# TravisWheelerLab/AvxWindowFmIndex

Hardware: AMD Instinct MI355X
Metric: Mkmers/sec located, GRCh38 nucleotide index (higher is better)
Workload: dtype u64

## Files before the change

### avxwindowfmindex_amd/_lib.py

```python
import ctypes as C
import os
import subprocess

_HERE = os.path.dirname(os.path.abspath(__file__))
LIB_PATH = os.environ.get("AWFM_LIB_PATH") or os.path.join(_HERE, "libawfmindex_amd.so")
_LIB = None

AwFmAlphabetAmino, AwFmAlphabetDna, AwFmAlphabetRna = 1, 2, 3
AwFmSuccess, AwFmFileReadOkay, AwFmFileWriteOkay = 1, 2, 3
AwFmGeneralFailure = -1
AwFmIllegalPositionError = -6
AwFmUnsupportedVersionError = -2
AwFmFileReadFail = -11

API_SYMBOLS = [
    "awFmCreateIndex", "awFmCreateIndexFromFasta", "awFmDeallocIndex", "awFmWriteIndexToFile",
    "awFmReadIndexFromFile", "awFmCreateKmerSearchList", "awFmDeallocKmerSearchList", "awFmParallelSearchLocate",
    "awFmParallelSearchCount", "awFmFindSearchRangeForString", "awFmReadSequenceFromFile",
    "awFmCreateInitialQueryRange", "awFmCreateInitialQueryRangeFromChar",
    "awFmNucleotideIterativeStepBackwardSearch", "awFmAminoIterativeStepBackwardSearch",
    "awFmFindDatabaseHitPositions", "awFmFindDatabaseHitPositionSingle",
    "awFmGetLocalSequencePositionFromIndexPosition", "awFmNucleotideBacktraceReturnPreviousLetterIndex",
    "awFmAminoBacktraceReturnPreviousLetterIndex", "awFmGetHeaderStringFromSequenceNumber", "awFmSearchRangeLength",
    "awFmReturnCodeIsFailure", "awFmReturnCodeIsSuccess", "awFmGetNumSequences",
]
GPU_SYMBOLS = [
    "awfmGpuDeviceCount", "awfmGpuLastError", "awfmGpuIndexCreate", "awfmGpuIndexDestroy", "awfmGpuIndexAcquire", "awfmGpuIndexAcquireAll",
    "awfmGpuIndexRelease", "awfmGpuIndexDeviceBytes", "awfmGpuIndexDevice", "awfmGpuIndexSetKernel", "awfmGpuIndexSetWide", "awfmGpuIndexIsWide", "awfmGpuLastBatchStatus", "awfmGpuIndexSetDeepSeed", "awfmGpuIndexSetDenseSa", "awfmGpuPinnedBuffer", "awfmGpuLocateHostWindows", "awfmGpuLocateWindow", "awfmGpuAosLock",
    "awfmGpuAosUnlock", "awfmGpuSearch", "awfmGpuSearchHits", "awfmGpuSearchHitsSparse", "awfmGpuIndexSetOrdered", "awfmGpuSearchHitsIsOrdered", "awfmGpuLastOrderedKernelMs", "awfmGpuLastOrderedKernelIsLookup", "awfmGpuLastOrderedKept", "awfmGpuLastSecondWindow",
    "awfmGpuScanScratchBytes", "awfmGpuHitOffsets", "awfmGpuHitOffsetsFromCounts", "awfmGpuLocate", "awfmGpuCountHost", "awfmGpuLocateHost",
    "awfmGpuCreateIndex", "awfmGpuSearchTally", "awfmGpuSynthText", "awfmGpuSynthRandomQueries", "awfmGpuSynthPlantedQueries",
    "awfmGpuSynthMixedLengths", "awfmGpuSynthMixedQueries", "awfmGpuSynthGenomeText", "awfmGpuSynthPlantedQueriesClean",
    "awfmPackKmers", "awfmGpuPackKmers", "awfmGpuUnpackKmers", "awfmGpuHostAlloc", "awfmGpuHostFree", "awfmGpuStreamPacked",
    "awfmGpuStreamChars", "awfmGpuCountPackedHost", "awfmGpuLocatePackedHost", "awfmGpuIndexSetPairImage", "awfmGpuIndexHasPairImage",
    "awfmGpuSearchHitsPacked", "awfmGpuLocateTo", "awfmGpuSearchHitsLineTally", "awfmGpuIndexDeepSeedK", "awfmGpuSearchHitsCompact", "awfmGpuCompactHits", "awfmGpuSortHits",
    "awfmGpuStreamPackedSparse", "awfmGpuStreamCharsSparse", "awfmGpuSearchHitsInOrder", "awfmGpuSearchHitsInOrderCounts",
    "awfmGpuSortHitsOnDevice", "awfmGpuHitOffsetsOnDevice", "awfmGpuLocateOnDevice", "awfmGpuLastOrderedSearchKernelMs", "awfmGpuOrderedKernelLog", "awfmGpuIndexDeepSeedBuildSeconds", "awfmGpuIndexDeepSeedTransientBytes", "awfmGpuIndexHasDenseSa", "awfmGpuIndexDenseSaBuildSeconds", "awfmGpuIndexLengthTableBytes", "awfmGpuIndexLengthTableBuildSeconds", "awfmGpuMixedLookupLineTally",
    "awfmGpuListLocateOnDevice", "awfmGpuLastLookupFront", "awfmGpuLastSearchWasExactLookup", "awfmGpuSynthPlantedQueriesUnique", "awfmGpuStreamRetire", "awfmGpuIndexDescribe", "awfmGpuIndexDeepSeedAllocSeconds", "awfmGpuAosLastStages", "awfmHostCopyGBs",
    "awfmLocalPositions", "awfmGpuIndexSetRecordTable", "awfmGpuIndexNumRecords", "awfmGpuLocalPositions", "awfmGpuLocateHostLocal",
    "awfmLongestSuffixMatches", "awfmGpuLongestSuffixMatches", "awfmOneSubstitutionSearch", "awfmGpuOneSubstitutionSearch",
    "awfmReadCandidates", "awfmGpuReadCandidates", "awfmGpuReadCandidatesScratchBytes",
    "awfmReadChains", "awfmGpuReadChains", "awfmGpuReadChainsScratchBytes",
    "awfmGpuIndexSetText", "awfmGpuIndexTextLength", "awfmTextWindows", "awfmGpuTextWindows", "awfmVerifyChains", "awfmGpuVerifyChains",
    "awfmAlignChains", "awfmGpuAlignChainsScratchBytes", "awfmGpuAlignChains",
    "awfmAlignChainsAffine", "awfmGpuAlignChainsAffineScratchBytes", "awfmGpuAlignChainsAffine",
    "awfmScoreChainsAffine", "awfmGpuScoreChainsAffine",
    "awfmScoreWindowsAffine", "awfmGpuScoreWindowsAffineScratchBytes", "awfmGpuScoreWindowsAffine",
    "awfmGpuOrderBuckets", "awfmGpuOrderKmers", "awfmGpuSearchOrderedRecords", "awfmGpuSearchOrderedRecordsCounts", "awfmGpuSearchGeneralRecords", "awfmGpuMergeBucketRuns",
]
CHUNK_SINK = C.CFUNCTYPE(C.c_int, C.c_void_p, C.c_uint64, C.c_uint64, C.POINTER(C.c_uint32), C.POINTER(C.c_uint64), C.c_uint64)


SPARSE_CHUNK_SINK = C.CFUNCTYPE(C.c_int, C.c_void_p, C.c_uint64, C.c_uint64, C.c_uint64, C.POINTER(C.c_uint32), C.POINTER(C.c_uint64),
                                C.POINTER(C.c_uint64), C.c_uint64)
HIT_WINDOW_SINK = C.CFUNCTYPE(C.c_int, C.c_void_p, C.c_uint64, C.c_uint64, C.c_uint64, C.c_uint64, C.POINTER(C.c_uint64))


class AwFmIndexConfiguration(C.Structure):
    _fields_ = [("suffixArrayCompressionRatio", C.c_uint8), ("kmerLengthInSeedTable", C.c_uint8),
                ("alphabetType", C.c_int), ("keepSuffixArrayInMemory", C.c_bool), ("storeOriginalSequence", C.c_bool)]


class AwFmCompressedSuffixArray(C.Structure):
    _fields_ = [("valueBitWidth", C.c_uint8), ("values", C.POINTER(C.c_uint8)), ("compressedByteLength", C.c_uint64)]


class AwFmSearchRange(C.Structure):
    _fields_ = [("startPtr", C.c_uint64), ("endPtr", C.c_uint64)]


class AwFmCandidateInputs(C.Structure):
    _fields_ = [("readSeedOffsets", C.c_void_p), ("numSeeds", C.c_uint64), ("seedEnds", C.c_void_p), ("seedLengths", C.c_void_p),
                ("fixedLength", C.c_uint32), ("hitOffsets", C.c_void_p), ("numHits", C.c_uint64), ("positions", C.c_void_p),
                ("sequenceNumbers", C.c_void_p)]


class AwFmCandidateOutputs(C.Structure):
    _fields_ = [("sequences", C.c_void_p), ("diagonals", C.c_void_p), ("votes", C.c_void_p), ("diagonalSpans", C.c_void_p),
                ("readBegins", C.c_void_p), ("readEnds", C.c_void_p), ("numCandidates", C.c_void_p), ("keptHits", C.c_void_p),
                ("numOverflowed", C.c_void_p)]


# ... 84 lines not shown
        import torch
    except Exception:
        pass
    L = C.CDLL(LIB_PATH, mode=C.RTLD_GLOBAL)
    IP, LP = C.POINTER(AwFmIndex), C.POINTER(AwFmKmerSearchList)
    RP = C.POINTER(AwFmSearchRange)
    vp, u64 = C.c_void_p, C.c_uint64
    sig = {
        "awFmCreateIndex": (C.c_int, [C.POINTER(IP), C.POINTER(AwFmIndexConfiguration), vp, C.c_size_t, C.c_char_p]),
        "awFmCreateIndexFromFasta": (C.c_int, [C.POINTER(IP), C.POINTER(AwFmIndexConfiguration), C.c_char_p, C.c_char_p]),
        "awFmDeallocIndex": (None, [IP]),
        "awFmWriteIndexToFile": (C.c_int, [IP, vp, u64, C.c_char_p]),
        "awFmReadIndexFromFile": (C.c_int, [C.POINTER(IP), C.c_char_p, C.c_bool]),
        "awFmCreateKmerSearchList": (LP, [C.c_size_t]),
        "awFmDeallocKmerSearchList": (None, [LP]),
        "awFmParallelSearchLocate": (C.c_int, [IP, LP, C.c_uint32]),
        "awFmParallelSearchCount": (None, [IP, LP, C.c_uint32]),
        "awFmFindSearchRangeForString": (AwFmSearchRange, [IP, C.c_char_p, C.c_size_t]),
        "awFmReadSequenceFromFile": (C.c_int, [IP, C.c_size_t, C.c_size_t, C.c_char_p]),
        "awFmCreateInitialQueryRange": (AwFmSearchRange, [IP, C.c_char_p, u64]),
        "awFmCreateInitialQueryRangeFromChar": (AwFmSearchRange, [IP, C.c_char]),
        "awFmNucleotideIterativeStepBackwardSearch": (None, [IP, RP, C.c_uint8]),
        "awFmAminoIterativeStepBackwardSearch": (None, [IP, RP, C.c_uint8]),
        "awFmFindDatabaseHitPositions": (C.POINTER(u64), [IP, RP, C.POINTER(C.c_int)]),
        "awFmFindDatabaseHitPositionSingle": (u64, [IP, u64, C.POINTER(C.c_int)]),
        "awFmNucleotideBacktraceReturnPreviousLetterIndex": (C.c_uint8, [IP, C.POINTER(u64)]),
        "awFmAminoBacktraceReturnPreviousLetterIndex": (C.c_uint8, [IP, C.POINTER(u64)]),
        "awFmGetLocalSequencePositionFromIndexPosition": (C.c_int, [IP, C.c_size_t, C.POINTER(C.c_size_t),
                                                                   C.POINTER(C.c_size_t)]),
        "awFmGetHeaderStringFromSequenceNumber": (C.c_int, [IP, C.c_size_t, C.POINTER(C.c_char_p), C.POINTER(C.c_size_t)]),
        "awFmSearchRangeLength": (C.c_size_t, [RP]),
        "awFmReturnCodeIsFailure": (C.c_bool, [C.c_int]),
        "awFmReturnCodeIsSuccess": (C.c_bool, [C.c_int]),
        "awFmGetNumSequences": (C.c_uint32, [IP]),
        "awfmGpuDeviceCount": (C.c_int, []),
        "awfmGpuLastError": (C.c_char_p, []),
        "awfmGpuIndexCreate": (C.c_int, [IP, C.c_int, C.POINTER(vp)]),
        "awfmGpuIndexDestroy": (None, [vp]),
        "awfmGpuIndexAcquire": (vp, [IP]),
        "awfmGpuIndexAcquireAll": (C.c_int, [IP, C.POINTER(vp), C.c_int]),
        "awfmGpuIndexRelease": (None, [IP]),
        "awfmGpuIndexDeviceBytes": (u64, [vp]),
        "awfmGpuIndexDevice": (C.c_int, [vp]),
        "awfmGpuIndexSetKernel": (None, [vp, C.c_int]),
        "awfmGpuIndexSetWide": (None, [vp, C.c_int]),
        "awfmGpuIndexIsWide": (C.c_int, [vp]),
        "awfmGpuLastBatchStatus": (C.c_int, []),
        "awfmGpuIndexSetOrdered": (None, [vp, C.c_int]),
        "awfmGpuSearchHitsIsOrdered": (C.c_int, [vp, C.c_int, C.c_uint32, u64]),
        "awfmGpuLastOrderedKernelMs": (C.c_double, [vp]),
        "awfmGpuLastOrderedKernelIsLookup": (C.c_int, [vp]),
        "awfmGpuLastOrderedKept": (C.c_uint64, [vp]),
        "awfmGpuLastSecondWindow": (None, [vp, C.POINTER(C.c_uint64 * 2)]),
        "awfmGpuIndexSetDeepSeed": (C.c_int, [vp, C.c_uint]),
        "awfmGpuIndexSetDenseSa": (C.c_int, [vp, C.c_int]),
        "awfmGpuIndexSetPairImage": (C.c_int, [vp, C.c_int]),
        "awfmGpuIndexHasPairImage": (C.c_int, [vp]),
        "awfmGpuIndexDeepSeedK": (C.c_uint, [vp]),
        "awfmGpuIndexDeepSeedBuildSeconds": (C.c_double, [vp]),
        "awfmGpuIndexDeepSeedTransientBytes": (u64, [vp]),
        "awfmGpuIndexHasDenseSa": (C.c_int, [vp]),
        "awfmGpuIndexDenseSaBuildSeconds": (C.c_double, [vp]),
        "awfmGpuIndexLengthTableBytes": (u64, [vp]),
        "awfmGpuIndexLengthTableBuildSeconds": (C.c_double, [vp]),
        "awfmGpuMixedLookupLineTally": (C.c_int, [vp, vp, vp, u64, C.POINTER(u64 * 8)]),
        "awfmGpuSearch": (C.c_int, [vp, vp, vp, C.c_uint32, u64, vp, vp, vp]),
        "awfmGpuSearchHits": (C.c_int, [vp, vp, vp, C.c_uint32, u64, vp, vp, vp]),
        "awfmGpuSearchHitsSparse": (C.c_int, [vp, vp, vp, C.c_uint32, u64, vp, vp, vp]),
        "awfmGpuSearchHitsCompact": (C.c_int, [vp, vp, vp, C.c_uint32, u64, C.c_int, vp, vp, C.c_uint32, vp, vp]),
        "awfmGpuCompactHits": (C.c_int, [vp, vp, vp, u64, vp, vp, vp, vp, C.c_uint32, vp, vp]),
        "awfmGpuSearchHitsInOrder": (C.c_int, [vp, vp, vp, C.c_uint32, u64, C.c_int, vp, vp, vp]),
        "awfmGpuSearchHitsInOrderCounts": (C.c_int, [vp, vp, vp, C.c_uint32, u64, C.c_int, vp, vp, vp, vp]),
        "awfmGpuOrderBuckets": (C.c_uint32, [vp, C.c_uint32, u64]),
        "awfmGpuOrderKmers": (C.c_int, [vp, vp, C.c_uint32, u64, u64, u64, vp, vp, vp]),
        "awfmGpuSearchOrderedRecords": (C.c_int, [vp, vp, vp, C.c_uint32, C.c_uint32, C.c_uint32, u64, vp, vp, vp]),
        "awfmGpuSearchOrderedRecordsCounts": (C.c_int, [vp, vp, vp, C.c_uint32, C.c_uint32, C.c_uint32, u64, vp, vp, vp, vp]),
        "awfmGpuMergeBucketRuns": (C.c_int, [vp, vp, vp, vp, C.c_uint32, C.c_uint32, C.c_uint32, C.c_uint32, vp, vp, vp]),
        "awfmGpuSearchGeneralRecords": (C.c_int, [vp, vp, C.c_uint32, u64, u64, u64, vp, vp, vp, vp, vp]),
        "awfmGpuSortHits": (C.c_int, [vp, vp, vp, C.c_uint32, vp]),
        "awfmGpuSortHitsOnDevice": (C.c_int, [vp, vp, vp, C.c_uint32, vp, u64, vp]),
        "awfmGpuListLocateOnDevice": (C.c_int, [vp, vp, vp, C.c_uint32, vp, u64, vp, vp, vp, u64, vp, vp]),
        "awfmGpuLastLookupFront": (C.c_int, [vp]),
        "awfmGpuLastSearchWasExactLookup": (C.c_int, [vp]),
        "awfmGpuStreamRetire": (None, [vp, vp]),
        "awfmGpuIndexDescribe": (C.c_int, [vp, C.c_char_p, C.c_int]),
        "awfmGpuIndexDeepSeedAllocSeconds": (C.c_double, [vp]),
        "awfmGpuAosLastStages": (None, [C.POINTER(C.c_double * 10)]),
        "awfmHostCopyGBs": (C.c_double, [C.c_uint32, u64]),
        "awfmGpuHitOffsetsOnDevice": (C.c_int, [vp, vp, vp, u64, vp, vp, vp]),
        "awfmGpuLocateOnDevice": (C.c_int, [vp, vp, vp, u64, u64, vp, vp]),
        "awfmGpuLastOrderedSearchKernelMs": (C.c_double, [vp]),
        "awfmGpuOrderedKernelLog": (C.c_int, [vp, C.POINTER(C.c_double), C.POINTER(C.c_double), C.c_int]),
        "awfmGpuScanScratchBytes": (u64, [u64]),
        "awfmGpuHitOffsets": (C.c_int, [vp, vp, u64, vp, vp, C.POINTER(u64), vp]),
        "awfmGpuHitOffsetsFromCounts": (C.c_int, [vp, vp, u64, vp, vp, C.POINTER(u64), vp]),
        "awfmGpuLocate": (C.c_int, [vp, vp, vp, u64, u64, vp, vp]),
        "awfmGpuLocateTo": (C.c_int, [vp, vp, vp, u64, u64, vp, vp, vp]),
        "awfmGpuLocateWindow": (C.c_int, [vp, vp, vp, u64, u64, u64, u64, vp, vp, vp]),
        "awfmGpuLocateHostWindows": (C.c_int, [vp, vp, vp, C.c_uint32, u64, vp, vp, HIT_WINDOW_SINK, vp]),
        "awfmGpuCountHost": (C.c_int, [vp, vp, vp, C.c_uint32, u64, vp, vp]),
        "awfmGpuLocateHost": (C.c_int, [vp, vp, vp, C.c_uint32, u64, vp, vp, C.POINTER(C.POINTER(u64))]),
        "awfmLocalPositions": (C.c_int, [IP, vp, u64, vp, vp, C.POINTER(u64), C.c_uint]),
        "awfmLongestSuffixMatches": (C.c_int, [IP, vp, vp, vp, C.c_uint32, u64, C.c_uint32, vp, vp, vp, C.c_uint]),
        "awfmGpuLongestSuffixMatches": (C.c_int, [vp, vp, vp, vp, C.c_uint32, u64, C.c_uint32, vp, vp, vp, vp]),
        "awfmOneSubstitutionSearch": (C.c_int, [IP, vp, vp, C.c_uint32, u64, C.c_int, vp, vp, vp, u64, vp, vp, vp, C.c_uint]),
        "awfmGpuOneSubstitutionSearch": (C.c_int, [vp, vp, vp, C.c_uint32, u64, C.c_int, vp, vp, vp, u64, vp, vp, vp, vp]),
# ... 77 lines not shown
```

### avxwindowfmindex_amd/api.py

```python
import ctypes as C
import os

import numpy as np

from . import _lib
from ._lib import (AwFmAlphabetAmino, AwFmAlphabetDna, AwFmAlphabetRna, AwFmFileReadOkay, AwFmFileWriteOkay,
                   AwFmIllegalPositionError, AwFmSuccess, AwFmUnsupportedVersionError)

ILLEGAL_SEQUENCE = 0xFFFFFFFF


class AwFmError(RuntimeError):
    def __init__(self, what, rc):
        msg = _lib.lib().awfmGpuLastError().decode(errors="replace")
        super().__init__(f"{what} failed with AwFmReturnCode {rc}" + (f": {msg}" if msg else ""))
        self.rc = rc


def _check(what, rc, ok=(AwFmSuccess, AwFmFileReadOkay, AwFmFileWriteOkay)):
    if rc not in ok:
        raise AwFmError(what, rc)
    return rc


# ... 745 lines not shown
            _check("awfmGpuIndexCreate", L.awfmGpuIndexCreate(index.ptr, device, C.byref(h)))
            self.handle = h
        self.index = index

    @classmethod
    def acquire_all(cls, index, max_handles=8):
        L = _lib.lib()
        if L.awfmGpuDeviceCount() <= 0:
            raise RuntimeError("no HIP device: the search path is GPU only (no CPU fallback)")
        handles = (C.c_void_p * max_handles)()
        n = L.awfmGpuIndexAcquireAll(index.ptr, handles, max_handles)
        out = []
        for h in handles[:n]:
            g = cls.__new__(cls)
            g.owned, g.handle, g.index = False, C.c_void_p(h), index
            out.append(g)
        return out

    @property
    def device_bytes(self):
        return int(_lib.lib().awfmGpuIndexDeviceBytes(self.handle))

    def set_deep_seed(self, deep_k):
        _check("awfmGpuIndexSetDeepSeed", _lib.lib().awfmGpuIndexSetDeepSeed(self.handle, deep_k))

    @property
    def deep_seed_k(self):
        return int(_lib.lib().awfmGpuIndexDeepSeedK(self.handle))

    @property
    def deep_seed_build(self):
        L = _lib.lib()
        return float(L.awfmGpuIndexDeepSeedBuildSeconds(self.handle)), int(L.awfmGpuIndexDeepSeedTransientBytes(self.handle))

    @property
    def deep_seed_alloc_s(self):
        return float(_lib.lib().awfmGpuIndexDeepSeedAllocSeconds(self.handle))

    def set_dense_sa(self, enable=True):
        _check("awfmGpuIndexSetDenseSa", _lib.lib().awfmGpuIndexSetDenseSa(self.handle, int(bool(enable))))

    @property
    def has_dense_sa(self):
        return bool(_lib.lib().awfmGpuIndexHasDenseSa(self.handle))

    @property
    def dense_sa_build_s(self):
        return float(_lib.lib().awfmGpuIndexDenseSaBuildSeconds(self.handle))

    @property
    def length_tables(self):
        return (int(_lib.lib().awfmGpuIndexLengthTableBytes(self.handle)), float(_lib.lib().awfmGpuIndexLengthTableBuildSeconds(self.handle)))

    def mixed_lookup_line_tally(self, d_chars, d_offsets, n):
        out = (C.c_uint64 * 8)()
        _check("awfmGpuMixedLookupLineTally", _lib.lib().awfmGpuMixedLookupLineTally(self.handle, d_chars, d_offsets, n, C.byref(out)))
        keys = ("length_table_lines", "deep_table_lines", "pair_level_lines", "nuc_level_lines", "kmers_alive_after_the_table",
                "kmers_with_hits", "general_kmers", "block_reads_executed")
        return {k: int(v) for k, v in zip(keys, out)}

    def set_pair_image(self, enable=True):
        _check("awfmGpuIndexSetPairImage", _lib.lib().awfmGpuIndexSetPairImage(self.handle, int(bool(enable))))

    @property
    def has_pair_image(self):
        return bool(_lib.lib().awfmGpuIndexHasPairImage(self.handle))

    def set_kernel(self, kernel):
        _lib.lib().awfmGpuIndexSetKernel(self.handle, kernel)

    def set_wide(self, wide=True):
        _lib.lib().awfmGpuIndexSetWide(self.handle, int(bool(wide)))

    @property
    def is_wide(self):
        return bool(_lib.lib().awfmGpuIndexIsWide(self.handle))

    def set_record_table(self, ends):
        ends = np.ascontiguousarray(ends, dtype=np.uint64)
        _check("awfmGpuIndexSetRecordTable", _lib.lib().awfmGpuIndexSetRecordTable(self.handle, ends.ctypes.data if ends.size else None,
                                                                                   ends.size))

    @property
    def num_records(self):
        return int(_lib.lib().awfmGpuIndexNumRecords(self.handle))

    def local_positions(self, d_positions, capacity, d_seq, d_local, d_num_positions=0, d_num_illegal=0, stream=0):
        _check("awfmGpuLocalPositions", _lib.lib().awfmGpuLocalPositions(self.handle, d_positions or None, capacity, d_num_positions or None,
                                                                         d_seq or None, d_local or None, d_num_illegal or None, stream or None))

    def read_candidates(self, inputs, num_reads, outputs, d_scratch, max_hits_per_seed=0, band=0, min_votes=1, max_candidates=4, stream=0):
        _check("awfmGpuReadCandidates", _lib.lib().awfmGpuReadCandidates(
            self.handle, C.byref(inputs), num_reads, max_hits_per_seed, band, min_votes, max_candidates, C.byref(outputs),
            d_scratch or None, stream or None))

    def read_chains(self, inputs, num_reads, d_sequences, d_diagonals, d_spans, outputs, d_scratch, max_hits_per_seed=0, band=0,
                    max_candidates=4, lookback=CHAINS_MAX_LOOKBACK, gap_penalty=0, stream=0):
        _check("awfmGpuReadChains", _lib.lib().awfmGpuReadChains(
            self.handle, C.byref(inputs), num_reads, max_hits_per_seed, band, max_candidates, d_sequences or None, d_diagonals or None,
            d_spans or None, lookback, gap_penalty, C.byref(outputs), d_scratch or None, stream or None))

    def set_text(self, text):
        if text is None:
            t = np.zeros(0, np.uint8)
        else:
            t = np.frombuffer(text, np.uint8) if isinstance(text, (bytes, bytearray)) else np.ascontiguousarray(text, dtype=np.uint8)
# ... 268 lines not shown

    def describe(self):
        import ctypes as C
        buf = C.create_string_buffer(2048)
        _lib.lib().awfmGpuIndexDescribe(self.handle, buf, 2048)
        return buf.value.decode()

    def stream_retire(self, stream):
        _lib.lib().awfmGpuStreamRetire(self.handle, stream or None)

    def last_lookup_front(self):
        return int(_lib.lib().awfmGpuLastLookupFront(self.handle))

    def last_search_was_exact_lookup(self):
        return bool(_lib.lib().awfmGpuLastSearchWasExactLookup(self.handle))

    def list_locate_on_device(self, d_hit_kmers, d_hit_ranges, capacity, d_num_hits, n, d_sorted_kmers, d_sorted_ranges, d_hit_offsets,
                              capacity_hits, d_positions, stream=0):
        _check("awfmGpuListLocateOnDevice", _lib.lib().awfmGpuListLocateOnDevice(
            self.handle, d_hit_kmers, d_hit_ranges, capacity, d_num_hits, n, d_sorted_kmers, d_sorted_ranges, d_hit_offsets,
            capacity_hits, d_positions or None, stream or None))

    def hit_offsets_on_device(self, d_counts, d_ranges, n, d_hit_offsets, d_scratch, stream=0):
        _check("awfmGpuHitOffsetsOnDevice", _lib.lib().awfmGpuHitOffsetsOnDevice(self.handle, d_counts or None, d_ranges or None, n,
                                                                                 d_hit_offsets, d_scratch, stream or None))

    def locate_on_device(self, d_ranges, d_hit_offsets, n, capacity_hits, d_positions, stream=0):
        _check("awfmGpuLocateOnDevice", _lib.lib().awfmGpuLocateOnDevice(self.handle, d_ranges, d_hit_offsets, n, capacity_hits,
                                                                         d_positions, stream or None))

    def ordered_kernel_log(self, max_entries=1024):
        front = (C.c_double * max_entries)()
        kern = (C.c_double * max_entries)()
        n = _lib.lib().awfmGpuOrderedKernelLog(self.handle, front, kern, max_entries)
        return [(front[i], kern[i]) for i in range(n)]

    def last_ordered_search_kernel_ms(self):
        return float(_lib.lib().awfmGpuLastOrderedSearchKernelMs(self.handle))

    def search_hits_is_ordered(self, has_offsets, fixed_length, n):
        return bool(_lib.lib().awfmGpuSearchHitsIsOrdered(self.handle, int(bool(has_offsets)), fixed_length, n))

    def last_ordered_kernel_ms(self):
        return float(_lib.lib().awfmGpuLastOrderedKernelMs(self.handle))

    def last_ordered_kept(self):
        return int(_lib.lib().awfmGpuLastOrderedKept(self.handle))

    def last_second_window(self):
        out = (C.c_uint64 * 2)()
        _lib.lib().awfmGpuLastSecondWindow(self.handle, C.byref(out))
        return int(out[0]), int(out[1])

    def last_ordered_kernel_is_lookup(self):
        return bool(_lib.lib().awfmGpuLastOrderedKernelIsLookup(self.handle))

    def set_ordered(self, mode):
        _lib.lib().awfmGpuIndexSetOrdered(self.handle, mode)

    def search_tally(self, d_chars, d_offsets, fixed_length, n):
        out = (C.c_uint64 * 4)()
        _check("awfmGpuSearchTally", _lib.lib().awfmGpuSearchTally(self.handle, d_chars, d_offsets or None, fixed_length,
                                                                   n, C.byref(out)))
        return {"seeded": int(out[0]), "steps": int(out[1]), "blocks": int(out[2]), "chars": int(out[3])}

    def search_hits_line_tally(self, d_chars, d_offsets, fixed_length, n):
        out = (C.c_uint64 * 8)()
        _check("awfmGpuSearchHitsLineTally", _lib.lib().awfmGpuSearchHitsLineTally(self.handle, d_chars, d_offsets or None,
                                                                                   fixed_length, n, C.byref(out)))
        keys = ("seed_table_lines", "deep_table_lines", "pair_level_lines", "nuc_level_lines", "ordered_kmers",
                "record_bytes_per_kmer", "kmers_with_hits", "general_kmers")
        return {k: int(v) for k, v in zip(keys, out)}

    def hit_offsets(self, d_ranges, n, d_hit_offsets, d_scratch, stream=0):
        total = C.c_uint64(0)
        _check("awfmGpuHitOffsets", _lib.lib().awfmGpuHitOffsets(self.handle, d_ranges, n, d_hit_offsets, d_scratch,
                                                                 C.byref(total), stream or None))
        return int(total.value)

    def hit_offsets_from_counts(self, d_counts, n, d_hit_offsets, d_scratch, stream=0):
        total = C.c_uint64(0)
        _check("awfmGpuHitOffsetsFromCounts", _lib.lib().awfmGpuHitOffsetsFromCounts(
            self.handle, d_counts, n, d_hit_offsets, d_scratch, C.byref(total), stream or None))
        return int(total.value)

    def locate(self, d_ranges, d_hit_offsets, n, total_hits, d_positions, stream=0):
        _check("awfmGpuLocate", _lib.lib().awfmGpuLocate(self.handle, d_ranges, d_hit_offsets, n, total_hits,
                                                         d_positions, stream or None))

    def locate_window(self, d_ranges, d_hit_offsets, query_begin, query_end, hit_begin, hit_end, d_positions, stream=0):
        _check("awfmGpuLocateWindow", _lib.lib().awfmGpuLocateWindow(self.handle, d_ranges, d_hit_offsets, query_begin, query_end,
                                                                     hit_begin, hit_end, d_positions, d_positions, stream or None))

    @staticmethod
    def scan_scratch_bytes(n):
        return int(_lib.lib().awfmGpuScanScratchBytes(n))

    def destroy(self):
        if self.handle:
            if self.owned:
                _lib.lib().awfmGpuIndexDestroy(self.handle)
            self.handle = None

    def __del__(self):
        try:
            self.destroy()
# ... 3 lines not shown
```

### avxwindowfmindex_amd/csrc/awfm_device.h

```cpp
#ifndef AWFM_DEVICE_H
#define AWFM_DEVICE_H

#include <hip/hip_runtime.h>

#include <atomic>
#include <cstdlib>
#include <cstring>
#include <mutex>
#include <shared_mutex>
#include <thread>
#include <vector>
#include <string>

#include "awfm_internal.h"

void awfmGpuSetError(const char *what);
void awfmGpuSetHipError(const char *what, hipError_t e);

namespace {

inline void setError(const char *what, hipError_t e) { awfmGpuSetHipError(what, e); }
inline void setError(const char *what) { awfmGpuSetError(what); }

#define AWFM_HIP_TRY(call, failRc)                      \
// ... 699 lines not shown
      if (half) {
        const unsigned pm = kAminoTables.planeMask[letter];
        for (unsigned j = 0; j < 4; j++) {
          Piece lo, hi;
          lo.x = planeWord(0, j);
          lo.y = planeWord(1, j);
          lo.z = planeWord(2, j);
          lo.w = planeWord(3, j);
          hi.x = planeWord(4, j);
          hi.y = hi.z = hi.w = 0;
          count += __popc(aminoOccSlice(lo, hi, pm & 0xFFu, pm >> 8));
        }
      }
      count -= super[(blk >> (kAminoSuperShift - kBlockShift)) * kAminoSuperStride + letter];
    }
    c16[s] = (unsigned)count & 0xFFFFu;
  }
  out[(blk * kSlices + k) * 2ull] = make_uint4(b[0], b[1], b[2], b[3]);
  out[(blk * kSlices + k) * 2ull + 1ull] = make_uint4(b[4], c16[0] | (c16[1] << 16), c16[2] | (c16[3] << 16), c16[4] | (c16[5] << 16));
  unsigned sentinelBits = ~(b[0] | b[1] | b[2] | b[3] | b[4]);
  while (sentinelBits) {
    const unsigned bit = (unsigned)(__ffs((int)sentinelBits) - 1);
    sentinelBits &= sentinelBits - 1u;
    const unsigned long long pos = (blk << kBlockShift) + k * 32u + bit;
    if (pos < bwtLength) *sentinelPos = pos;
  }
}

}

struct AwFmGpuIndex;

struct AwFmGpuImage {
  DevIndex dev{};
  void *dBlocks = nullptr;
  void *dSuper = nullptr;
  void *dSeed = nullptr;
  void *dSa = nullptr;
  void *dPrefix = nullptr;
  void *dDeepSeed = nullptr;
  uint64_t deepSeedBytes = 0;
  double deepSeedBuildSeconds = 0.0;
  double deepSeedAllocSeconds = 0.0;
  uint64_t deepSeedTransientBytes = 0;
  void *dDeepBig = nullptr;
  std::mutex lengthMutex;
  void *dLengthTable = nullptr;
  unsigned lengthDepths = 0;
  bool lengthTried = false;
  unsigned lengthRetryIn = 0;
  void *dLengthBig = nullptr;
  uint64_t lengthTableBytes = 0;
  double lengthTableBuildSeconds = 0.0;
  void *dDenseSa = nullptr;
  bool denseWide = false;
  uint64_t denseSaBytes = 0;
  double denseSaBuildSeconds = 0.0;
  void *dPairBlocks = nullptr, *dPairSuper = nullptr, *dPairSuper32 = nullptr, *dPairC = nullptr;
  uint64_t pairBytes = 0;
  std::string accelNotes;
  uint64_t deviceBytes = 0;
  uint64_t numBlocks = 0;
  std::mutex joinMutex;
  std::thread accelThread;
  std::atomic<int> accelState{0};
  struct PendingAccel {
    void *deepTable = nullptr, *deepBig = nullptr;
    uint64_t deepBytes = 0, deepBigBytes = 0, deepTransient = 0;
    unsigned deepK = 0, deepFormat = 0, deepNext = 0, numDeepBig = 0;
    double deepSeconds = 0.0, deepAllocSeconds = 0.0;
    void *dense = nullptr;
    bool denseWide = false;
    uint64_t denseBytes = 0;
    double denseSeconds = 0.0;
    std::string notes;
  } pendingAccel;
  std::mutex streamMutex;
  struct AwFmGpuStreamState *streamState = nullptr;
  std::mutex handlesMutex;
  std::vector<AwFmGpuIndex *> handles;
  std::shared_mutex recordMutex;
  DevRecords records{};
  void *dRecords = nullptr;
  uint64_t recordBytes = 0;
  bool recordsInLds = false;
  unsigned recordLdsBytes = 0;
  unsigned recordGrid = 0;
  void *dText = nullptr;
  uint64_t textLength = 0;
  uint64_t textBytes = 0;
};

struct AwFmGpuIndex {
  AwFmGpuImage *image = nullptr;
  int lane = 0;
  int device = 0;
  bool amino = false;
  int numCUs = 256;
  AwFmGpuKernel kernel = AWFM_GPU_KERNEL_AUTO;
  bool forceWide = false;
  std::mutex workMutex;
  void *dWork = nullptr;
  size_t workBytes = 0;
  void *dHits = nullptr;
  size_t hitsBytes = 0;
  mutable uint64_t hitBudgetAuto = 0;
  void *dSparse = nullptr;
  size_t sparseBytes = 0;
  hipEvent_t windowEvent[2] = {nullptr, nullptr};
  int orderMode = -1;
  std::mutex orderMutex;
  struct StreamGate {
    hipEvent_t done = nullptr;
    bool recorded = false;
    bool pending = false;
    hipStream_t lastStream = nullptr;
    std::thread::id lastThread;
  };
  struct OrderSlot {
    void *mem = nullptr;
    size_t bytes = 0;
    StreamGate gate;
    unsigned long long lastUse = 0;
    int prepParity = -1;
  };
  static constexpr int kOrderSlots = 2;
  OrderSlot orderSlot[kOrderSlots];
  unsigned long long orderUses = 0;
  int orderCur = 0;
  int orderPrevParity = -1;
  void *dOrder = nullptr;
  size_t orderBytes = 0;
  hipEvent_t orderDoneEvent = nullptr;
  bool orderDoneArmed = false;
  StreamGate sparseGate;
  hipEvent_t orderTiming[4] = {nullptr, nullptr, nullptr, nullptr};
  bool orderTimedFront = false, orderTimedKernel = false;
  struct OrderLogEntry {
    hipEvent_t ev[4] = {nullptr, nullptr, nullptr, nullptr};
    bool front = false, kernel = false;
  };
  static constexpr unsigned kOrderLogMax = 1024;
  std::vector<OrderLogEntry> orderLog;
  unsigned long long orderLogCount = 0;
  int orderLookup = 0;
  const unsigned *orderSampleAt = nullptr;
  unsigned orderSamples = 0;
  bool orderLookupFused = false;
  const unsigned *orderFusedKeptAt = nullptr;
  const unsigned *orderKeptAt = nullptr;
  struct LookupPredict {
    unsigned long long *verdictHost = nullptr;
    unsigned searches = 0;
    int lastFront = -1;
    unsigned lastJudged = 0;
    unsigned holdoff = 0;
    unsigned holdoffNext = 8;
    unsigned agreed = 0;
  } predict;
  int lastSearchExact = 0;
  std::mutex aosMutex;
  void *pinned[4] = {nullptr, nullptr, nullptr, nullptr};
  size_t pinnedBytes[4] = {0, 0, 0, 0};
};

inline const char *awfmGpuDiag(const char *key) {
  const char *env = awfmKnob(AWFM_KNOB_DIAG);
  if (!env) return nullptr;
  static thread_local char value[32];
  const size_t keyLen = strlen(key);
  for (const char *at = env; *at;) {
    const char *end = strchr(at, ',');
    const size_t len = end ? (size_t)(end - at) : strlen(at);
    if (len > keyLen && !strncmp(at, key, keyLen) && at[keyLen] == '=') {
      const size_t n = len - keyLen - 1 < sizeof(value) - 1 ? len - keyLen - 1 : sizeof(value) - 1;
      memcpy(value, at + keyLen + 1, n);
      value[n] = 0;
      return value;
    }
    at += len + (end ? 1 : 0);
  }
  return nullptr;
}

inline uint64_t awfmDeviceBlocks(uint64_t bwtLength) { return 2 * awfmNumBlocks(bwtLength); }
inline uint64_t awfmDeviceBlockBytes(bool amino) { return amino ? 128 : 64; }
inline unsigned awfmSuperShift(bool amino, uint64_t bwtLength) {
  if (amino) return kAminoSuperShift;
  if (const char *env = awfmGpuDiag("nuc_super_shift")) {
    if (!strcmp(env, "auto")) {
      unsigned shift = 13;
      while (((bwtLength - 1) >> shift) + 1 > 48) shift++;
      return shift < kNucSuperShift ? shift : kNucSuperShift;
    }
    const int v = atoi(env);
    if (v >= 13 && v < (int)kNucSuperShift) return (unsigned)v;
  }
  return kNucSuperShift;
}
inline uint64_t awfmNumSuper(uint64_t bwtLength, bool amino, unsigned superShift) {
  (void)amino;
  return ((bwtLength - 1) >> superShift) + 1;
}
// ... 125 lines not shown
```

### avxwindowfmindex_amd/csrc/awfm_gpu_image.hip

```cpp
#include <hip/hip_runtime.h>
#include <cstdio>
#include <cstdlib>
#include <cstring>
#include <mutex>
#include <string>
#include <system_error>
#include <vector>

#include "awfm_device.h"
#include "awfm_search_kernel.h"
#include "awfm_locate_kernel.h"

thread_local hipStream_t awfmGpuSetupStream = nullptr;
static thread_local std::string tlsError;
void awfmGpuSetError(const char *what) { tlsError = what; }
void awfmGpuSetHipError(const char *what, hipError_t e) { tlsError = std::string(what) + ": " + hipGetErrorString(e); }


namespace {

std::mutex tableMutex;
struct ImageEntry {
  const AwFmIndex *index;
  AwFmGpuIndex *handle;
// ... 335 lines not shown
    if (!take(h->aosMutex) || !take(h->workMutex) || !take(h->orderMutex)) return;
  held = true;
}
AwFmGpuExclusive::~AwFmGpuExclusive() {
  while (!locked.empty()) {
    locked.back()->unlock();
    locked.pop_back();
  }
}

void awfmGpuAdoptAccelerators(AwFmGpuImage *image, bool wait) {
  if (image->accelState.load() == 0) return;
  if (wait) joinBuilder(image);
  else if (image->accelState.load() != 2) return;
  AwFmGpuExclusive section(image, wait);
  if (!section.held || image->accelState.load() != 2) return;
  joinBuilder(image);
  AwFmGpuImage::PendingAccel &from = image->pendingAccel;
  if (from.deepTable) installDeepSeed(image, &from);
  if (from.dense) {
    image->dDenseSa = from.dense;
    image->denseWide = from.denseWide;
    image->denseSaBytes = from.denseBytes;
    image->denseSaBuildSeconds = from.denseSeconds;
    from.dense = nullptr;
  }
  image->accelNotes += from.notes;
  from.notes.clear();
  image->accelState.store(0);
}
extern "C" {

void awfmGpuIndexDestroy(AwFmGpuIndex *g) {
  if (!g) return;
  AwFmGpuImage *image = g->image;
  if (g->lane) {
    std::lock_guard<std::mutex> lock(image->handlesMutex);
    for (size_t i = 0; i < image->handles.size(); i++)
      if (image->handles[i] == g) {
        image->handles.erase(image->handles.begin() + (long)i);
        break;
      }
  } else {
    joinBuilder(image);
  }
  {
    DeviceGuard guard(g->device);
    if (!g->lane) {
      if (image->pendingAccel.deepTable) (void)hipFree(image->pendingAccel.deepTable);
      if (image->pendingAccel.deepBig) (void)hipFree(image->pendingAccel.deepBig);
      if (image->pendingAccel.dense) (void)hipFree(image->pendingAccel.dense);
      awfmGpuStreamStateFree(image);
      void *owned[] = {image->dBlocks, image->dSuper, image->dSeed, image->dSa, image->dPrefix, image->dDeepSeed, image->dDeepBig,
                       image->dDenseSa, image->dLengthTable, image->dLengthBig, image->dPairBlocks, image->dPairSuper,
                       image->dPairSuper32, image->dPairC, image->dRecords, image->dText};
      for (void *p : owned)
        if (p) (void)hipFree(p);
    }
    if (g->dWork) (void)hipFree(g->dWork);
    if (g->dHits) (void)hipFree(g->dHits);
    for (auto &slot : g->orderSlot) {
      if (slot.mem) (void)hipFree(slot.mem);
      if (slot.gate.done) (void)hipEventDestroy(slot.gate.done);
    }
    if (g->dSparse) (void)hipFree(g->dSparse);
    if (g->sparseGate.done) (void)hipEventDestroy(g->sparseGate.done);
    for (auto &entry : g->orderLog)
      for (int i = 0; i < 4; i++)
        if (entry.ev[i]) (void)hipEventDestroy(entry.ev[i]);
    for (int i = 0; i < 2; i++)
      if (g->windowEvent[i]) (void)hipEventDestroy(g->windowEvent[i]);
    for (int i = 0; i < 4; i++)
      if (g->pinned[i]) (void)hipHostFree(g->pinned[i]);
    if (g->predict.verdictHost) (void)hipHostFree(g->predict.verdictHost);
  }
  if (!g->lane) delete image;
  delete g;
}

static int aosDevices(int *devs, int maxOut) {
  int n = 0;
  const char *env = awfmKnob(AWFM_KNOB_DEVICES);
  if (env && !strcmp(env, "all")) {
    const int count = awfmGpuDeviceCount();
    for (int d = 0; d < count && n < maxOut; d++) devs[n++] = d;
  } else if (env && *env) {
    for (const char *c = env; *c && n < maxOut;) {
      devs[n++] = atoi(c);
      while (*c && *c != ',') c++;
      if (*c == ',') c++;
    }
  }
  if (n == 0) {
    devs[n++] = -1;
    for (int lane = 1; lane < 3 && n < maxOut; lane++) devs[n++] = -1;
  }
  return n;
}

static AwFmGpuIndex *addLane(AwFmGpuIndex *primary) {
  AwFmGpuIndex *g = new AwFmGpuIndex();
  g->image = primary->image;
  g->device = primary->device;
  g->amino = primary->amino;
  g->numCUs = primary->numCUs;
  g->kernel = primary->kernel;
  g->forceWide = primary->forceWide;
// ... 38 lines not shown
  return n;
}

AwFmGpuIndex *awfmGpuIndexAcquire(const struct AwFmIndex *index) {
  AwFmGpuIndex *g = nullptr;
  if (awfmGpuIndexAcquireAll(index, &g, 1) != 1) return nullptr;
  awfmGpuAdoptAccelerators(g->image, true);
  return g;
}

void awfmGpuIndexRelease(const struct AwFmIndex *index) {
  std::vector<AwFmGpuIndex *> doomed;
  {
    std::lock_guard<std::mutex> lock(tableMutex);
    for (size_t i = 0; i < imageTable.size();) {
      if (imageTable[i].index == index) {
        doomed.push_back(imageTable[i].handle);
        imageTable.erase(imageTable.begin() + (long)i);
      } else {
        i++;
      }
    }
  }
  for (AwFmGpuIndex *g : doomed)
    if (g->lane) awfmGpuIndexDestroy(g);
  for (AwFmGpuIndex *g : doomed)
    if (!g->lane) awfmGpuIndexDestroy(g);
}

void *awfmGpuPinnedBuffer(AwFmGpuIndex *g, int slot, uint64_t bytes) {
  if (!g || slot < 0 || slot > 3) return nullptr;
  if (bytes <= g->pinnedBytes[slot]) return g->pinned[slot];
  DeviceGuard guard(g->device);
  if (g->pinned[slot]) (void)hipHostFree(g->pinned[slot]);
  g->pinned[slot] = nullptr;
  g->pinnedBytes[slot] = 0;
  const size_t want = bytes + bytes / 4 + 4096;
  if (hipHostMalloc(&g->pinned[slot], want, hipHostMallocDefault) != hipSuccess) {
    setError("awfmGpuPinnedBuffer: hipHostMalloc failed");
    g->pinned[slot] = nullptr;
    return nullptr;
  }
  g->pinnedBytes[slot] = want;
  return g->pinned[slot];
}
void awfmGpuAosLock(AwFmGpuIndex *g) {
  if (g) g->aosMutex.lock();
}
void awfmGpuAosUnlock(AwFmGpuIndex *g) {
  if (g) g->aosMutex.unlock();
}

static uint64_t imageBytes(const AwFmGpuImage *image) {
  return image->deviceBytes + image->deepSeedBytes + image->denseSaBytes + image->pairBytes + image->lengthTableBytes + image->recordBytes + image->textBytes;
}
uint64_t awfmGpuIndexDeviceBytes(const AwFmGpuIndex *g) { return g && !g->lane ? imageBytes(g->image) : 0; }

static enum AwFmReturnCode applyDeepSeed(AwFmGpuIndex *g, unsigned deepK);

enum AwFmReturnCode awfmGpuIndexSetDeepSeed(AwFmGpuIndex *g, unsigned deepK) {
  if (!g) {
    setError("awfmGpuIndexSetDeepSeed: null image");
    return AwFmNullPtrError;
  }
  if (g->lane) {
    setError("awfmGpuIndexSetDeepSeed: set it on the primary image, not on a lane");
    return AwFmIllegalPositionError;
  }
  awfmGpuAdoptAccelerators(g->image, true);
  DeviceGuard guard(g->device);
  AwFmGpuExclusive section(g->image);
  return applyDeepSeed(g, deepK);
}

static enum AwFmReturnCode buildDeepSeed(AwFmGpuIndex *g, unsigned deepK, AwFmGpuImage::PendingAccel *to) {
  void *table = nullptr, *big = nullptr;
  uint64_t bytes = 0, peak = 0;
  unsigned format = 0, numBig = 0;
  struct timespec t0, t1;
  clock_gettime(CLOCK_MONOTONIC, &t0);
  if (!awfmGpuBuildDeepSeedTable(g, deepK, &table, &bytes, &peak, &to->deepAllocSeconds, &format, &big)) return AwFmGeneralFailure;
  const int next = awfmGpuDeepSeedAddNext(g, table, deepK, format, &big, &numBig);
  (void)awfmGpuSetupSync();
  clock_gettime(CLOCK_MONOTONIC, &t1);
  if (next < 0) {
    (void)hipFree(table);
    if (big) (void)hipFree(big);
    return AwFmGeneralFailure;
  }
  to->deepTable = table;
  to->deepBig = big;
  to->deepBytes = bytes;
  to->deepBigBytes = !big ? 0u
                     : format == 2u ? ((g->image->dev.bwtLength >> (g->amino ? kAminoWideBigShift : kDeepWideBigShift)) + 2u) * 8u
                                    : ((g->image->dev.bwtLength >> (g->amino ? kAminoDeepBigShift : kDeepBigShift)) + 5u) * 4u;
  to->deepTransient = peak > bytes ? peak - bytes : 0;
  to->deepK = deepK;
  to->deepFormat = format;
  to->deepNext = next > 0 ? 1u : 0u;
  to->numDeepBig = numBig;
  to->deepSeconds = (double)(t1.tv_sec - t0.tv_sec) + 1e-9 * (double)(t1.tv_nsec - t0.tv_nsec);
  if (awfmKnob(AWFM_KNOB_VERBOSE))
    fprintf(stderr, "[awfm deeper table] depth %u, entry format %u: %.2f GB in %.2f s; next-step bits %s; %u entries with long ranges\n", deepK, format,
            (double)bytes * 1e-9, to->deepSeconds, next > 0 ? "yes" : "no", numBig);
  return AwFmSuccess;
}
static void installDeepSeed(AwFmGpuImage *image, AwFmGpuImage::PendingAccel *from) {
  image->dDeepSeed = from->deepTable;
  image->dDeepBig = from->deepBig;
  image->deepSeedBytes = from->deepBytes + from->deepBigBytes;
  image->deepSeedBuildSeconds = from->deepSeconds;
  image->deepSeedAllocSeconds = from->deepAllocSeconds;
  image->deepSeedTransientBytes = from->deepTransient;
  image->dev.deepSeed = (const ulonglong2 *)from->deepTable;
  image->dev.deepNarrow = from->deepFormat;
  image->dev.deepNext = from->deepNext;
  image->dev.numDeepBig = from->numDeepBig;
  image->dev.deepBigBySp = (const unsigned *)from->deepBig;
  image->dev.deepK = from->deepTable ? from->deepK : 0u;
  from->deepTable = from->deepBig = nullptr;
}

static enum AwFmReturnCode applyDeepSeed(AwFmGpuIndex *g, unsigned deepK) {
  AwFmGpuImage *image = g->image;
  (void)hipDeviceSynchronize();
  if (image->dDeepSeed) (void)hipFree(image->dDeepSeed);
  if (image->dDeepBig) (void)hipFree(image->dDeepBig);
  {
    std::lock_guard<std::mutex> lock(image->lengthMutex);
    if (image->dLengthTable) (void)hipFree(image->dLengthTable);
    if (image->dLengthBig) (void)hipFree(image->dLengthBig);
    image->dLengthTable = nullptr;
    image->dLengthBig = nullptr;
    image->lengthDepths = 0;
    image->lengthTableBytes = 0;
    image->lengthTried = false;
  }
  AwFmGpuImage::PendingAccel built;
  enum AwFmReturnCode rc = AwFmSuccess;
  if (deepK != 0) {
    image->dev.deepSeed = nullptr;
    image->dev.deepK = 0;
    rc = buildDeepSeed(g, deepK, &built);
  }
  installDeepSeed(image, &built);
  return rc;
}

static unsigned chooseDeepSeedK(const AwFmGpuIndex *g, std::string &notes);
static enum AwFmReturnCode applyDeepSeedFromEnv(AwFmGpuIndex *g) {
  const unsigned deepK = chooseDeepSeedK(g, g->image->accelNotes);
  if (deepK == 0) return AwFmSuccess;
  DeviceGuard guard(g->device);
  return applyDeepSeed(g, deepK);
}
static unsigned chooseDeepSeedK(const AwFmGpuIndex *g, std::string &notes) {
  int deepK = 0;
  if (const char *env = awfmKnob(g->amino ? AWFM_KNOB_AMINO_DEEP_SEED_K : AWFM_KNOB_DEEP_SEED_K)) {
    deepK = atoi(env);
  } else if (g->amino) {
// ... 39 lines not shown
    (void)awfmGpuApplyPairImage(g, false);
    g->image->accelNotes += "pair image: not built (no device memory for 1 byte per position); ";
  }
  return rc;
}

enum AwFmReturnCode awfmGpuIndexSetPairImage(AwFmGpuIndex *g, int enable) {
  if (!g) {
    setError("awfmGpuIndexSetPairImage: null image");
    return AwFmNullPtrError;
  }
  if (g->lane) {
    setError("awfmGpuIndexSetPairImage: set it on the primary image, not on a lane");
    return AwFmIllegalPositionError;
  }
  awfmGpuAdoptAccelerators(g->image, true);
  DeviceGuard guard(g->device);
  AwFmGpuExclusive section(g->image);
  const enum AwFmReturnCode rc = awfmGpuApplyPairImage(g, enable != 0);
  if (rc != AwFmSuccess) (void)awfmGpuApplyPairImage(g, false);
  return rc;
}
int awfmGpuIndexHasPairImage(const AwFmGpuIndex *g) { return g && g->image->dev.pairBlocks ? 1 : 0; }
unsigned awfmGpuIndexDeepSeedK(const AwFmGpuIndex *g) { return g ? g->image->dev.deepK : 0u; }
double awfmGpuIndexDeepSeedAllocSeconds(const AwFmGpuIndex *g) { return g ? g->image->deepSeedAllocSeconds : 0.0; }
double awfmGpuIndexDeepSeedBuildSeconds(const AwFmGpuIndex *g) { return g ? g->image->deepSeedBuildSeconds : 0.0; }
uint64_t awfmGpuIndexDeepSeedTransientBytes(const AwFmGpuIndex *g) { return g ? g->image->deepSeedTransientBytes : 0; }

int awfmGpuIndexDevice(const AwFmGpuIndex *g) { return g ? g->device : -1; }
void awfmGpuIndexSetKernel(AwFmGpuIndex *g, enum AwFmGpuKernel kernel) {
  if (g) g->kernel = kernel;
}
int awfmGpuIndexIsWide(const AwFmGpuIndex *g) { return g && !awfmImageNarrow(g) ? 1 : 0; }
void awfmGpuIndexSetWide(AwFmGpuIndex *g, int wide) {
  if (!g) return;
  if (g->lane) {
    g->forceWide = wide != 0;
    return;
  }
  std::lock_guard<std::mutex> lock(g->image->handlesMutex);
  for (AwFmGpuIndex *h : g->image->handles) h->forceWide = wide != 0;
}


int awfmGpuIndexDescribe(const AwFmGpuIndex *g, char *out, int outBytes) {
  if (!g || !out || outBytes <= 0) return 0;
  const AwFmGpuImage *image = g->image;
  std::string text = std::string(g->amino ? "amino" : "nucleotide") + " image of " + std::to_string(image->dev.bwtLength) + " positions, " +
                     std::to_string(imageBytes(image)) + " bytes on device " + std::to_string(g->device) + ": ";
  if (!g->amino) text += image->dev.pairBlocks ? "pair image yes; " : "pair image no; ";
  text += image->dev.deepK ? "deeper table depth " + std::to_string(image->dev.deepK) + (image->dev.deepNext ? " with next-step bits; " : "; ") : "deeper table no; ";
  text += image->dDenseSa ? "full suffix array yes; " : "full suffix array no; ";
  if (!g->amino) text += image->dLengthTable ? "tables per k-mer length 1.." + std::to_string(image->lengthDepths) + "; " : "tables per k-mer length not built (the first large mixed-length batch builds them); ";
  text += awfmGpuDescribeRecordTable(image);
  text += awfmGpuDescribeText(image);
  if (!image->accelNotes.empty()) text += "notes: " + image->accelNotes;
  while (!text.empty() && (text.back() == ' ' || text.back() == ';')) text.pop_back();
  const int n = (int)text.size() < outBytes - 1 ? (int)text.size() : outBytes - 1;
  memcpy(out, text.data(), (size_t)n);
  out[n] = 0;
  return (int)text.size();
}
uint64_t awfmGpuIndexLengthTableBytes(const AwFmGpuIndex *g) { return g ? g->image->lengthTableBytes : 0; }
double awfmGpuIndexLengthTableBuildSeconds(const AwFmGpuIndex *g) { return g ? g->image->lengthTableBuildSeconds : 0.0; }

}
```

### avxwindowfmindex_amd/csrc/awfm_gpu_ordered.hip

```cpp
#include <cstring>
#include <cstdio>
#include <cstdlib>
#include <cstddef>

#include <hip/hip_runtime.h>
#include <hip/hip_ext.h>
#include <rocprim/rocprim.hpp>

#include "awfm_ordered_kernel.h"
#include "awfm_amino_lookup_kernel.h"
#include "awfm_count_order_kernel.h"

namespace {

inline size_t alignUp256(size_t v) { return (v + 255) / 256 * 256; }

__global__ void __launch_bounds__(256) fillSparseKernel(unsigned *__restrict__ kmers, ulonglong2 *__restrict__ ranges, unsigned cap,
                                                        unsigned *__restrict__ count) {
  const unsigned i = blockIdx.x * 256u + threadIdx.x;
  if (i < cap) {
    kmers[i] = 0xFFFFFFFFu;
    ranges[i] = make_ulonglong2(1ull, 0ull);
  }
  if (i == 0) *count = 0u;
}
inline hipError_t fillSparseList(const SparseOut *sparse, hipStream_t s) {
  if (!sparse || !sparse->count) return hipSuccess;
  hipLaunchKernelGGL(fillSparseKernel, dim3((sparse->cap + 255u) / 256u), dim3(256), 0, s, sparse->kmers, sparse->ranges, sparse->cap, sparse->count);
  return hipGetLastError();
}
constexpr size_t kOrderCounterBytes = 131072;
static_assert(256 + 8 * kTicketGroups * 8 * 256 <= kOrderCounterBytes, "ticket counters");

template <class Kernel>
unsigned residentGrid(const AwFmGpuIndex *g, Kernel kernel, size_t dynamicLds = 0, int threads = kThreads) {
  int perCU = 0;
  if (hipOccupancyMaxActiveBlocksPerMultiprocessor(&perCU, kernel, threads, dynamicLds) != hipSuccess || perCU < 1) perCU = 4;
  if (perCU > 8) perCU = 8;
  return (unsigned)g->numCUs * (unsigned)perCU;
}

inline bool pairSteps(const AwFmGpuIndex *g) { return g->image->dev.pairBlocks != nullptr; }

template <bool NARROW, bool VARLEN, bool PAIR = false, bool TOUCH = false, bool BUCKET = false, bool LIST = false>
enum AwFmReturnCode launchOrderedKernel(AwFmGpuIndex *g, hipStream_t s, uint32_t len, unsigned depth, const ulonglong2 *table,
                                        unsigned long long nq, const void *recs, const unsigned *generalCount, ulonglong2 *rng,
                                        uint32_t *dCounts, const OrderTouch *touch = nullptr, const unsigned *bucketStart = nullptr,
                                        const BucketFormat bucketFmt = BucketFormat(), const SparseOut *sparse = nullptr,
                                        const unsigned *skipSampleAlive = nullptr, unsigned skipSamples = 0u) {
  constexpr int G = 4;
  const bool superInLds = PAIR && NARROW && awfmPairSuperInLds(g);
  const size_t lds = superInLds ? (size_t)g->image->dev.numPairSuper * 64u : 0u;
  DevIndex dev = g->image->dev;
  dev.pairSuperInLds = superInLds ? 1u : 0u;
  constexpr int threads = orderedThreads(PAIR);
  unsigned grid = residentGrid(g, orderedSearchKernel<G, NARROW, VARLEN, PAIR, TOUCH, BUCKET, LIST>, lds, threads);
  const unsigned long long blocks = (nq + threads / G - 1) / (threads / G);
  if (blocks < grid) grid = (unsigned)blocks;
  if (grid >= 8u) grid &= ~7u;
  const bool timed = g->orderTiming[2] != nullptr;
  OrderSkip<VARLEN> skip;
  if constexpr (VARLEN) {
    skip.sampleAlive = skipSampleAlive;
    skip.samples = skipSamples;
  }
  AWFM_LAUNCH_WITH_EVENTS((orderedSearchKernel<G, NARROW, VARLEN, PAIR, TOUCH, BUCKET, LIST>), dim3(grid ? grid : 1u), dim3(threads), (unsigned)lds, s,
                        timed ? g->orderTiming[2] : nullptr, timed ? g->orderTiming[3] : nullptr, dev, recs, nq, generalCount, len, depth, table,
                        rng, dCounts, (unsigned *)generalCount + 64, touch ? *touch : OrderTouch(), bucketStart, bucketFmt,
                        sparse ? *sparse : SparseOut(),
                        BUCKET ? 2u : 1u, skip);
  AWFM_HIP_TRY(hipGetLastError(), AwFmGeneralFailure);
  g->orderTimedKernel = timed;
  if (timed) g->orderLog[(g->orderLogCount - 1u) % AwFmGpuIndex::kOrderLogMax].kernel = true;
  return AwFmSuccess;
}

template <bool NARROW, bool CSR>
enum AwFmReturnCode launchLeftover(AwFmGpuIndex *g, hipStream_t s, const uint8_t *dChars, const unsigned long long *off, uint32_t len,
                                   unsigned long long nq, ulonglong2 *rng, uint32_t *dCounts, const void *recs, unsigned recordBytes,
                                   unsigned indexAt, const unsigned *leftCount, const SparseOut *sparse, bool last = true) {
  const unsigned grid = residentGrid(g, searchKernel<false, 4, CSR, false, NARROW, true>);
  AWFM_LAUNCH_WITH_EVENTS((searchKernel<false, 4, CSR, false, NARROW, true>), dim3(grid), dim3(kThreads), 0u, s, nullptr, last ? g->orderDoneEvent : nullptr,
                          g->image->dev, dChars, off, len, nq, rng, dCounts, (unsigned long long *)nullptr, (const unsigned char *)recs, recordBytes,
                          indexAt, nq, leftCount, sparse ? *sparse : SparseOut(), (const unsigned *)nullptr, 0u);
  AWFM_HIP_TRY(hipGetLastError(), AwFmGeneralFailure);
  if (last) g->orderDoneArmed = g->orderDoneEvent != nullptr;
  return AwFmSuccess;
}

template <bool NARROW, bool VARLEN>
enum AwFmReturnCode launchOrdered(AwFmGpuIndex *g, hipStream_t s, const uint8_t *dChars, const unsigned long long *off,
                                  uint32_t len, unsigned depth, const ulonglong2 *table, unsigned long long nq,
                                  const void *recs, const unsigned *generalCount, ulonglong2 *rng, uint32_t *dCounts,
                                  const OrderTouch *touch = nullptr, const SparseOut *sparse = nullptr,
                                  const unsigned *skipSampleAlive = nullptr, unsigned skipSamples = 0u) {
  enum AwFmReturnCode rc;
  const BucketFormat none = BucketFormat();
  if (touch)
    rc = pairSteps(g) ? launchOrderedKernel<NARROW, VARLEN, true, true>(g, s, len, depth, table, nq, recs, generalCount, rng, dCounts, touch)
                      : launchOrderedKernel<NARROW, VARLEN, false, true>(g, s, len, depth, table, nq, recs, generalCount, rng, dCounts, touch);
  else
    rc = pairSteps(g) ? launchOrderedKernel<NARROW, VARLEN, true>(g, s, len, depth, table, nq, recs, generalCount, rng, dCounts, nullptr, nullptr, none, sparse, skipSampleAlive, skipSamples)
                      : launchOrderedKernel<NARROW, VARLEN, false>(g, s, len, depth, table, nq, recs, generalCount, rng, dCounts, nullptr, nullptr, none, sparse, skipSampleAlive, skipSamples);
  if (rc != AwFmSuccess) return rc;
  return launchLeftover<NARROW, VARLEN>(g, s, dChars, off, len, nq, rng, dCounts, recs, (unsigned)sizeof(QueryRec), (unsigned)offsetof(QueryRec, index),
                                        generalCount, sparse);
}

template <bool NARROW>
enum AwFmReturnCode launchBucketed(AwFmGpuIndex *g, hipStream_t s, const uint8_t *dChars, uint32_t len, unsigned depth,
                                   const ulonglong2 *table, unsigned long long nq, const void *recs, const unsigned *bucketStart,
                                   const BucketFormat &fmt, const unsigned *generalCount, ulonglong2 *rng, uint32_t *dCounts,
                                   bool packed, const OrderTouch *touch, const SparseOut *sparse, bool countRecords = false) {
  const bool pair = pairSteps(g);
  enum AwFmReturnCode rc;
  if (touch)
    rc = pair ? launchOrderedKernel<NARROW, false, true, true, true>(g, s, len, depth, table, nq, recs, generalCount, rng, dCounts, touch, bucketStart, fmt)
              : launchOrderedKernel<NARROW, false, false, true, true>(g, s, len, depth, table, nq, recs, generalCount, rng, dCounts, touch, bucketStart, fmt);
  else if (sparse && sparse->count)
    rc = pair ? launchOrderedKernel<NARROW, false, true, false, true, true>(g, s, len, depth, table, nq, recs, generalCount, rng, dCounts, nullptr, bucketStart, fmt, sparse)
              : launchOrderedKernel<NARROW, false, false, false, true, true>(g, s, len, depth, table, nq, recs, generalCount, rng, dCounts, nullptr, bucketStart, fmt, sparse);
  else
    rc = pair ? launchOrderedKernel<NARROW, false, true, false, true>(g, s, len, depth, table, nq, recs, generalCount, rng, dCounts, nullptr, bucketStart, fmt, sparse)
              : launchOrderedKernel<NARROW, false, false, false, true>(g, s, len, depth, table, nq, recs, generalCount, rng, dCounts, nullptr, bucketStart, fmt, sparse);
  if (rc != AwFmSuccess || packed || countRecords) return rc;
  return launchLeftover<NARROW, false>(g, s, dChars, nullptr, len, nq, rng, dCounts, recs, 8u, 0u, generalCount, sparse);
}

}

static bool orderedApplies(const AwFmGpuIndex *g, bool hasOffsets, uint32_t fixedLength, unsigned long long nq,
                           unsigned *depthOut, const ulonglong2 **tableOut) {
  if (g->amino || nq >= 0xFFFFFFFFull || g->image->dev.seedK == 0 || g->image->dev.seedK >= 32 || g->image->dev.deepK >= 32) return false;
  if (!hasOffsets) {
    if (fixedLength == 0 || fixedLength > 32) return false;
    const bool deep = g->image->dev.deepK != 0 && fixedLength >= g->image->dev.deepK;
    const unsigned depth = deep ? g->image->dev.deepK : g->image->dev.seedK;
    if (fixedLength < depth) return false;
    if (depthOut) *depthOut = depth;
    if (tableOut) *tableOut = deep ? g->image->dev.deepSeed : g->image->dev.seed;
  }
  int mode = g->orderMode;
  if (mode < 0) {
    if (const char *env = awfmKnob(AWFM_KNOB_ORDERED)) mode = atoi(env) != 0;
  }
  if (mode < 0) {
    mode = nq >= (1ull << 23) && g->image->dev.bwtLength >= (1ull << 28);
  }
  return mode != 0;
}

int awfmGpuDeepSeedAddNext(AwFmGpuIndex *g, void *table, unsigned deepK, unsigned format, void **bigOut, unsigned *numBigOut) {
  *numBigOut = 0;
  if (!g || !table || format == 0u || deepK == 0) return 0;
  if (g->amino ? deepK > 7u : (!g->image->dev.pairBlocks || deepK > 16u)) return 0;
  if (awfmKnob(AWFM_KNOB_DEEP_NEXT) && atoi(awfmKnob(AWFM_KNOB_DEEP_NEXT)) == 0) return 0;
  DeviceGuard guard(g->device);
  if (format == 2u) {
    unsigned *dCount = nullptr;
    if (hipMalloc((void **)&dCount, 16) != hipSuccess) {
      (void)hipGetLastError();
      return 0;
    }
    unsigned numBig = 0;
    bool ok = awfmGpuSetupMemset(dCount, 0, 16) == hipSuccess;
    if (ok) {
      DevIndex dev = g->image->dev;
      dev.deepNarrow = 2u;
      dev.deepBigBySp = (const unsigned *)*bigOut;
      dev.pairSuperInLds = 0u;
      if (g->amino) {
        unsigned long long numEntries = 1;
        for (unsigned k = 0; k < deepK; k++) numEntries *= 20ull;
        const unsigned grid = residentGrid(g, aminoDeepNextKernel<false>, 0, kThreads);
        hipLaunchKernelGGL(aminoDeepNextKernel<false>, dim3(grid ? grid : 1u), dim3(kThreads), 0, awfmGpuSetupStream, dev, (uint2 *)table, numEntries, (unsigned *)nullptr, dCount);
      } else {
// ... 344 lines not shown
                          const unsigned *sampleAlive = nullptr, unsigned samples = 0u) {
  launchEncode4At<32u>(len, grid, lds, s, dChars, fmt, nq, codes, hist, binsPad, sampleAlive, samples);
}

template <unsigned K, bool NARROW>
static void launchLookupSearchAt(unsigned len, unsigned grid, size_t lds, hipStream_t s, const DevIndex &dev, const uint8_t *dChars,
                                 const BucketFormat &fmt, unsigned useNext, unsigned long long nq, unsigned long long *codes,
                                 unsigned *numbers, unsigned *shareCount, unsigned *hist, unsigned binsPad,
                                 const unsigned *sampleAlive, unsigned samples, ulonglong2 *rng, unsigned *dCounts,
                                 const SparseOut &sparse, unsigned *keptCounters, hipEvent_t start, hipEvent_t stop) {
  if (len == K)
    AWFM_LAUNCH_WITH_EVENTS((lookupSearchKernel<K, NARROW>), dim3(grid), dim3(256), (unsigned)lds, s, start, stop, dev, dChars, fmt, useNext, nq, codes,
                          numbers, shareCount, hist, binsPad, sampleAlive, samples, rng, dCounts, sparse, keptCounters);
  else if constexpr (K > 1u)
    launchLookupSearchAt<K - 1u, NARROW>(len, grid, lds, s, dev, dChars, fmt, useNext, nq, codes, numbers, shareCount, hist, binsPad, sampleAlive, samples,
                                         rng, dCounts, sparse, keptCounters, start, stop);
}

enum { kFrontBoth = 0, kFrontLookupOnly = 1, kFrontOrderedOnly = 2 };
constexpr unsigned kPredictHoldoff = 8, kPredictSamples = 16384, kPredictNumberMask = (1u << 22) - 1u;
static int predictFront(AwFmGpuIndex *g, unsigned fixedLength, unsigned chooseOf = kPredictSamples) {
  AwFmGpuIndex::LookupPredict &p = g->predict;
  if (const char *env = awfmKnob(AWFM_KNOB_LOOKUP_PREDICT))
    if (atoi(env) == 0) return kFrontBoth;
  if (!p.verdictHost) return kFrontBoth;
  const unsigned long long v = *(volatile unsigned long long *)p.verdictHost;
  const unsigned tag = (unsigned)(v >> 32), alive = (unsigned)v;
  const unsigned number = tag & kPredictNumberMask, front = (tag >> 22) & 3u, length = (tag >> 24) & 63u;
  if (number == 0u) return kFrontBoth;
  if (length != fixedLength) return p.holdoff ? (p.holdoff--, kFrontBoth) : kFrontBoth;
  const bool lookup = alive * 4u < chooseOf;
  if (number != p.lastJudged) {
    p.lastJudged = number;
    if ((front == kFrontLookupOnly && !lookup) || (front == kFrontOrderedOnly && lookup)) {
      p.holdoff = p.holdoffNext;
      p.holdoffNext = p.holdoffNext < 1024u ? 2u * p.holdoffNext : 1024u;
      p.agreed = 0;
    } else if (front != kFrontBoth && ++p.agreed >= 64u) {
      p.holdoffNext = kPredictHoldoff;
    }
  }
  if (p.holdoff) {
    p.holdoff--;
    return kFrontBoth;
  }
  return lookup ? kFrontLookupOnly : kFrontOrderedOnly;
}
static unsigned predictTag(AwFmGpuIndex *g, int front, unsigned fixedLength) {
  AwFmGpuIndex::LookupPredict &p = g->predict;
  p.searches = (p.searches + 1u) & kPredictNumberMask;
  if (p.searches == 0u) p.searches = 1u;
  p.lastFront = front;
  return p.searches | ((unsigned)front << 22) | ((fixedLength & 63u) << 24);
}

static int bucketedSearch(AwFmGpuIndex *g, hipStream_t s, const uint8_t *dChars, uint32_t fixedLength, unsigned depth,
                          const ulonglong2 *table, unsigned long long nq, ulonglong2 *rng, uint32_t *dCounts, bool packed,
                          bool rangesOfHitsOnly, const OrderTouch *touch, const BucketFormat &fmt, const SparseOut *sparse) {
  const unsigned bins = (1u << fmt.bucketBits) + 1u, binsPad = (bins + 3u) & ~3u;
  const size_t histAt = kOrderCounterBytes, cursorsAt = histAt + alignUp256((size_t)kShares * binsPad * 4u);
  const size_t startAt = cursorsAt + alignUp256((size_t)kShares * binsPad * 4u);
  const size_t codesAt = startAt + alignUp256((bins + 1u) * 4u), recsAt = codesAt + (packed ? 0u : alignUp256(nq * 8u));
  const bool narrow = awfmImageNarrow(g);
  const bool lookupCapable = !packed && !touch && table == g->image->dev.deepSeed && g->image->dev.deepNarrow != 0u &&
                             !(sparse && sparse->kmers && !sparse->count);
  const char *lookupEnv = awfmKnob(AWFM_KNOB_LOOKUP_FIRST);
  const bool lookupWanted = lookupCapable && (lookupEnv ? atoi(lookupEnv) != 0 : nq >= (1ull << 20));
  const size_t numbersAt = recsAt + alignUp256(nq * 8u);
  const unsigned countBuckets = countOrderBuckets(nq);
  const bool countRecords = !sparse && !touch && dCounts && !rng && countBuckets != 0u;
  constexpr unsigned countShift = kCountShift;
  const size_t countInAt = numbersAt + (lookupWanted ? alignUp256(nq * 4u) : 0u);
  const size_t countOutAt = countInAt + (countRecords ? alignUp256(nq * 8u) : 0u);
  const size_t total = countOutAt + (countRecords ? alignUp256(((size_t)countBuckets << countShift) * 8u) : 0u);
  if (orderBeginSlot(g, s) != hipSuccess) {
    setError("seed-order search: could not order the use of its scratch across streams");
    return -(int)AwFmGeneralFailure;
  }
  OrderSlotScope slotScope(g, s);
  if (!ensureOrderScratch(g, total)) return kOrderNoScratch;
  constexpr size_t kShareCountAt = 98304, kSampleAt = kShareCountAt + kShares * kShareCountStride * 4u;
  constexpr size_t kKeptAt = 102400;
  constexpr size_t kCountCursorsAt = 66048;
  static_assert(256 + 8 * kTicketGroups * 8 * 256 <= kCountCursorsAt && kCountCursorsAt + kCountBucketsMax * 4u <= kShareCountAt, "counter block");
  static_assert(256 + 8 * kTicketGroups * 8 * 256 <= kShareCountAt && kSampleAt + 4 <= kKeptAt && kKeptAt + kFusedCounters * 64u <= kOrderCounterBytes, "counter block");
#define BUCKET_TRY(call)                    \
  do {                                      \
    hipError_t e__ = (call);                \
    if (e__ != hipSuccess) {                \
      setError(#call, e__);                 \
      return -(int)AwFmGeneralFailure;      \
    }                                       \
  } while (0)
  uint8_t *w = (uint8_t *)g->dOrder;
  unsigned *generalCount = (unsigned *)w;
  unsigned *hist = (unsigned *)(w + histAt), *cursors = (unsigned *)(w + cursorsAt), *bucketStart = (unsigned *)(w + startAt);
  const unsigned long long *codes = packed ? (const unsigned long long *)dChars : (const unsigned long long *)(w + codesAt);
  unsigned long long *recs = (unsigned long long *)(w + recsAt);
  const unsigned long long perShare256 = (shareSize(nq) + 255ull) / 256ull;
  unsigned encodeGrid = (unsigned)(perShare256 * kShares < (unsigned long long)g->numCUs * 8u ? perShare256 * kShares : (unsigned long long)g->numCUs * 8u);
  encodeGrid = (encodeGrid + kShares - 1u) / kShares * kShares;
  unsigned *shareCount = (unsigned *)(w + kShareCountAt), *numbers = (unsigned *)(w + numbersAt);
  const unsigned useNext = g->image->dev.deepNext != 0u && pairSteps(g) && fixedLength >= depth + 2u ? 1u : 0u;
  constexpr unsigned kSamples = 16384;
  const bool forced = lookupWanted && lookupEnv && atoi(lookupEnv) == 1;
  bool bySample = lookupWanted && !forced;
// ... 80 lines not shown
          const unsigned long long tripsEach = (tripsPerShare + groupsPerShare - 1ull) / groupsPerShare;
          if (tripsEach <= 64ull) fusedGrid = (unsigned)((tripsPerShare + tripsEach - 1ull) / tripsEach) * kShares;
        }
      }
#define AWFM_LOOKUP_GO(NR)                                                                                                               \
  launchLookupSearchAt<32u, NR>(fixedLength, fusedGrid, lds, s, dev, dChars, fmt, useNext | (pairOff ? 2u : 0u) | (lookupOnly ? 4u : 0u) | secondBits, nq, \
                                (unsigned long long *)(w + codesAt), lookupOnly ? (unsigned *)recs : numbers, lookupOnly ? generalCount : shareCount, \
                                hist, binsPad, sampleAlive, kSamples, rng, dCounts, sparse ? *sparse : SparseOut(),                      \
                                (unsigned *)(w + kKeptAt), timed ? g->orderTiming[0] : nullptr, timed ? g->orderTiming[1] : nullptr)
      if (narrow) AWFM_LOOKUP_GO(true);
      else AWFM_LOOKUP_GO(false);
#undef AWFM_LOOKUP_GO
    }
    g->orderTimedFront = timed;
    if (timed) g->orderLog[(g->orderLogCount - 1u) % AwFmGpuIndex::kOrderLogMax].front = true;
    BUCKET_TRY(hipGetLastError());
  }
  if (lookupOnly) {
    enum AwFmReturnCode rc = AwFmSuccess;
    if (!packed)
      rc = narrow ? launchLeftover<true, false>(g, s, dChars, nullptr, fixedLength, nq, rng, dCounts, recs, 8u, 0u, generalCount, sparse)
                  : launchLeftover<false, false>(g, s, dChars, nullptr, fixedLength, nq, rng, dCounts, recs, 8u, 0u, generalCount, sparse);
    if (rc != AwFmSuccess) return -(int)rc;
    BUCKET_TRY(slotScope.end());
    return 1;
  }
  if (lookupFirst) {
  } else if (packed)
    hipLaunchKernelGGL((encodeCodesKernel<true>), dim3(encodeGrid), dim3(256), bins * 4u, s, dChars, fixedLength, fmt, nq,
                       (unsigned long long *)nullptr, hist, binsPad);
  else
    launchEncode4(fixedLength, encodeGrid, bins * 4u, s, dChars, fmt, nq, (unsigned long long *)(w + codesAt), hist, binsPad, sampleAlive, kSamples);
  BUCKET_TRY(hipGetLastError());
  hipLaunchKernelGGL(bucketScanSharesKernel, dim3(1), dim3(1024), 0, s, hist, bins, binsPad, bucketStart, generalCount, (unsigned)nq);
  BUCKET_TRY(hipGetLastError());
  const size_t partitionLds = (size_t)kPartitionTile * 8u + 3u * binsPad * 4u;
  static std::once_flag ldsOnce;
  static hipError_t ldsError = hipSuccess;
  std::call_once(ldsOnce, [] {
    ldsError = hipFuncSetAttribute((const void *)partitionKernel, hipFuncAttributeMaxDynamicSharedMemorySize,
                                   (int)(kPartitionTile * 8u + 3u * (((1u << kBucketBitsMax) + 4u) & ~3u) * 4u));
  });
  BUCKET_TRY(ldsError);
  const unsigned long long tilesPerShare = shareSize(nq) / kPartitionTile;
  unsigned partitionGrid = (unsigned)(tilesPerShare * kShares < (unsigned long long)g->numCUs ? tilesPerShare * kShares : (unsigned long long)g->numCUs);
  partitionGrid = (partitionGrid + kShares - 1u) / kShares * kShares;
  hipLaunchKernelGGL(partitionKernel, dim3(partitionGrid), dim3(kPartitionThreads), partitionLds, s, codes, fixedLength, fmt, nq,
                     (const unsigned *)hist, cursors, recs, packed ? 0u : 1u,
                     lookupFirst || bySample ? (const unsigned *)shareCount : (const unsigned *)nullptr,
                     lookupFirst || bySample ? (const unsigned *)numbers : (const unsigned *)nullptr, sampleAlive, kSamples);
  BUCKET_TRY(hipGetLastError());
  const SparseOut countOut{nullptr, 0u, (unsigned *)(w + countInAt), nullptr};
  const SparseOut *results = countRecords ? &countOut : sparse;
  const enum AwFmReturnCode rc =
      narrow ? launchBucketed<true>(g, s, dChars, fixedLength, depth, table, nq, recs, bucketStart, fmt, generalCount, rng, dCounts, packed, touch, results, countRecords)
                         : launchBucketed<false>(g, s, dChars, fixedLength, depth, table, nq, recs, bucketStart, fmt, generalCount, rng, dCounts, packed, touch, results, countRecords);
  if (rc != AwFmSuccess) return -(int)rc;
  if (countRecords) {
    const unsigned *ordered = bucketStart + (1u << fmt.bucketBits);
    unsigned *countCursors = (unsigned *)(w + kCountCursorsAt);
    const unsigned long long tiles = (nq + kCountScatterTile - 1ull) / kCountScatterTile;
    const unsigned scatterGrid = (unsigned)(tiles < (unsigned long long)g->numCUs * 8u ? tiles : (unsigned long long)g->numCUs * 8u);
    hipLaunchKernelGGL(countScatterKernel, dim3(scatterGrid ? scatterGrid : 1u), dim3(kCountScatterThreads), 0, s, (const uint2 *)(w + countInAt), ordered,
                       countBuckets, (uint2 *)(w + countOutAt), countCursors);
    BUCKET_TRY(hipGetLastError());
    static std::once_flag placeOnce;
    static hipError_t placeError = hipSuccess;
    std::call_once(placeOnce, [] {
      placeError = hipFuncSetAttribute((const void *)countPlaceKernel, hipFuncAttributeMaxDynamicSharedMemorySize, (int)((1u << kCountShift) * 4u));
    });
    BUCKET_TRY(placeError);
    hipLaunchKernelGGL(countPlaceKernel, dim3(countBuckets), dim3(kCountPlaceThreads), (size_t)(1u << kCountShift) * 4u, s, (const uint2 *)(w + countOutAt),
                       (const unsigned *)countCursors, nq, dCounts);
    BUCKET_TRY(hipGetLastError());
    if (!packed) {
      const enum AwFmReturnCode left = narrow ? launchLeftover<true, false>(g, s, dChars, nullptr, fixedLength, nq, rng, dCounts, recs, 8u, 0u, generalCount, nullptr)
                                              : launchLeftover<false, false>(g, s, dChars, nullptr, fixedLength, nq, rng, dCounts, recs, 8u, 0u, generalCount, nullptr);
      if (left != AwFmSuccess) return -(int)left;
    }
  }
  BUCKET_TRY(slotScope.end());
#undef BUCKET_TRY
  return 1;
}

int awfmGpuOrderedSearch(AwFmGpuIndex *g, hipStream_t s, const uint8_t *dChars, const unsigned long long *off,
                         uint32_t fixedLength, unsigned long long nq, ulonglong2 *rng, uint32_t *dCounts, bool packed,
                         bool rangesOfHitsOnly) {
  return orderedSearch(g, s, dChars, off, fixedLength, nq, rng, dCounts, packed, rangesOfHitsOnly, nullptr, nullptr, nullptr);
}

static const uint2 *ensureLengthTables(AwFmGpuIndex *g) {
  AwFmGpuImage *im = g->image;
  const unsigned need = im->dev.deepK - 1u;
  std::lock_guard<std::mutex> lock(im->lengthMutex);
  if (im->dLengthTable && im->lengthDepths >= need) return (const uint2 *)im->dLengthTable;
  if (im->lengthTried && (++im->lengthRetryIn & 63u) != 0u) return nullptr;
  im->lengthTried = true;
  {
    const uint64_t tableBytes = awfmLengthTableAt(need + 1u) * 8ull;
    size_t freeBytes = 0, totalBytes = 0;
    if (hipMemGetInfo(&freeBytes, &totalBytes) != hipSuccess || (uint64_t)freeBytes / 3u < tableBytes) {
      (void)hipGetLastError();
      return nullptr;
    }
  }
  struct timespec t0, t1;
  clock_gettime(CLOCK_MONOTONIC, &t0);
  void *table = nullptr;
// ... 436 lines not shown
    return AwFmAllocationFailure;
  }
  hipStream_t s = nullptr;
  unsigned long long *pairLines = bits + lengthWords + deepWords, *nucLines = pairLines + (uint64_t)levels * pairWords;
  unsigned long long *sums = nucLines + (uint64_t)levels * nucWords;
  const bool pairOff = !pairSteps(g);
  const unsigned useNext = (g->image->dev.deepNext != 0u && !pairOff ? 1u : 0u) | (pairOff ? 2u : 0u);
  hipError_t e = hipMemsetAsync(bits, 0, words * 8u, s);
  unsigned long long host[8] = {0};
  if (e == hipSuccess)
    e = awfmGpuLaunchMixedTally(g, s, lengthTable, dChars, (const unsigned long long *)dOffsets, (unsigned long long)numQueries, useNext, bits,
                                lengthWords, deepWords, pairWords, nucWords);
  if (e == hipSuccess) {
    const struct { const unsigned long long *from; uint64_t n; } parts[4] = {
        {bits, lengthWords}, {bits + lengthWords, deepWords}, {pairLines, (uint64_t)levels * pairWords}, {nucLines, (uint64_t)levels * nucWords}};
    for (int i = 0; i < 4 && e == hipSuccess; i++) {
      hipLaunchKernelGGL(popcountWordsKernel, dim3(2048), dim3(256), 0, s, parts[i].from, (unsigned long long)parts[i].n, sums + 3 + i);
      e = hipGetLastError();
    }
  }
  if (e == hipSuccess) e = hipMemcpyAsync(host, sums, sizeof host, hipMemcpyDeviceToHost, s);
  if (e == hipSuccess) e = hipStreamSynchronize(s);
  (void)hipFree(bits);
  if (e != hipSuccess) {
    setError("awfmGpuMixedLookupLineTally", e);
    return AwFmGeneralFailure;
  }
  tallyOut[0] = host[3];
  tallyOut[1] = host[4];
  tallyOut[2] = host[5];
  tallyOut[3] = host[6];
  tallyOut[4] = host[0];
  tallyOut[5] = host[1];
  tallyOut[6] = host[2];
  tallyOut[7] = host[7];
  return AwFmSuccess;
}

extern "C" enum AwFmReturnCode awfmGpuSearchHitsLineTally(AwFmGpuIndex *g, const uint8_t *dChars, const uint64_t *dOffsets,
                                                          uint32_t fixedLength, uint64_t numQueries, uint64_t tallyOut[8]) {
  if (!g || !dChars || !tallyOut) {
    setError("awfmGpuSearchHitsLineTally: null argument");
    return AwFmNullPtrError;
  }
  for (int i = 0; i < 8; i++) tallyOut[i] = 0;
  if (!awfmGpuSearchHitsIsOrdered(g, dOffsets != nullptr, fixedLength, numQueries)) {
    setError("awfmGpuSearchHitsLineTally: this batch does not take the seed-order path on this image");
    return AwFmUnsupportedVersionError;
  }
  DeviceGuard guard(g->device);
  const uint64_t seedWords = (g->image->dev.seedLen * 16u / 128u + 64u) / 64u;
  const uint64_t deepWords = g->image->dev.deepK ? ((1ull << (2u * g->image->dev.deepK)) * (g->image->dev.deepNarrow ? 8u : 16u) / 128u + 64u) / 64u : 1u;
  const uint64_t pairWords = (g->image->numBlocks + 64u) / 64u, nucWords = (g->image->numBlocks / 2u + 64u) / 64u;
  const uint64_t words = seedWords + deepWords + (uint64_t)kTouchLevels * (pairWords + nucWords) + 8u;
  unsigned long long *bits = nullptr;
  if (hipMalloc((void **)&bits, words * 8u) != hipSuccess) {
    (void)hipGetLastError();
    setError("awfmGpuSearchHitsLineTally: no device memory for the line bitmaps");
    return AwFmAllocationFailure;
  }
  hipStream_t s = nullptr;
  enum AwFmReturnCode rc = AwFmSuccess;
  OrderTouch touch;
  touch.seedLines = bits;
  touch.deepLines = touch.seedLines + seedWords;
  touch.pairLines = touch.deepLines + deepWords;
  touch.nucLines = touch.pairLines + (uint64_t)kTouchLevels * pairWords;
  touch.pairWords = pairWords;
  touch.nucWords = nucWords;
  unsigned long long *sums = touch.nucLines + (uint64_t)kTouchLevels * nucWords;
  touch.hits = sums;
  uint64_t recordBytes = 0;
  hipError_t e = hipMemsetAsync(bits, 0, words * 8u, s);
  if (e == hipSuccess) {
    const int did = orderedSearch(g, s, dChars, (const unsigned long long *)dOffsets, fixedLength, numQueries, nullptr, nullptr, false,
                                  false, &touch, &recordBytes, nullptr);
    if (did <= 0) rc = did < 0 ? (enum AwFmReturnCode)(-did) : AwFmGeneralFailure;
  }
  unsigned generalCount = 0;
  unsigned long long host[8] = {0};
  if (e == hipSuccess && rc == AwFmSuccess) {
    const struct { const unsigned long long *from; uint64_t n; } parts[4] = {
        {touch.seedLines, seedWords}, {touch.deepLines, deepWords}, {touch.pairLines, (uint64_t)kTouchLevels * pairWords},
        {touch.nucLines, (uint64_t)kTouchLevels * nucWords}};
    for (int i = 0; i < 4; i++)
      hipLaunchKernelGGL(popcountWordsKernel, dim3(1024), dim3(256), 0, s, parts[i].from, (unsigned long long)parts[i].n, sums + 1 + i);
    e = hipGetLastError();
    if (e == hipSuccess) e = hipMemcpyAsync(host, sums, sizeof(host), hipMemcpyDeviceToHost, s);
    if (e == hipSuccess) e = hipMemcpyAsync(&generalCount, g->dOrder, sizeof(generalCount), hipMemcpyDeviceToHost, s);
    if (e == hipSuccess) e = hipStreamSynchronize(s);
  }
  (void)hipFree(bits);
  if (e != hipSuccess) {
    setError("awfmGpuSearchHitsLineTally", e);
    return AwFmGeneralFailure;
  }
  if (rc != AwFmSuccess) return rc;
  tallyOut[0] = host[1];
  tallyOut[1] = host[2];
  tallyOut[2] = host[3];
  tallyOut[3] = host[4];
  tallyOut[4] = numQueries - generalCount;
  tallyOut[5] = recordBytes;
  tallyOut[6] = host[0];
  tallyOut[7] = generalCount;
  return AwFmSuccess;
}


namespace {
__global__ void __launch_bounds__(256) compactDenseKernel(const unsigned *__restrict__ counts, const ulonglong2 *__restrict__ ranges,
                                                          const unsigned long long *__restrict__ flagOffsets, unsigned long long n,
                                                          unsigned cap, unsigned *__restrict__ kmers, ulonglong2 *__restrict__ outRanges,
                                                          unsigned *__restrict__ count) {
  for (unsigned long long i = (unsigned long long)blockIdx.x * 256ull + threadIdx.x; i < n; i += (unsigned long long)gridDim.x * 256ull) {
    if (counts[i] != 0u) {
      const unsigned long long at = flagOffsets[i];
      if (at < cap) {
        kmers[at] = (unsigned)i;
        outRanges[at] = ranges[i];
      }
    }
  }
  if (blockIdx.x == 0 && threadIdx.x == 0) *count = (unsigned)(flagOffsets[n] < 0xFFFFFFFFull ? flagOffsets[n] : 0xFFFFFFFFull);
}
}

extern "C" enum AwFmReturnCode awfmGpuSearchHitsCompact(AwFmGpuIndex *g, const uint8_t *dChars, const uint64_t *dOffsets,
                                                        uint32_t fixedLength, uint64_t numQueries, int packed, uint32_t *dHitKmers,
                                                        struct AwFmSearchRange *dHitRanges, uint32_t capacity, uint32_t *dNumHits,
                                                        void *stream) {
  if (!g || !dChars || !dHitKmers || !dHitRanges || !dNumHits) {
    setError("awfmGpuSearchHitsCompact: null argument");
    return AwFmNullPtrError;
  }
  if (capacity == 0) {
    setError("awfmGpuSearchHitsCompact: the list needs a capacity");
    return AwFmIllegalPositionError;
  }
  if ((g->amino && (packed || dOffsets)) || (!g->amino && !(g->kernel == AWFM_GPU_KERNEL_AUTO || g->kernel == AWFM_GPU_KERNEL_GROUP4)) || (packed && dOffsets)) {
    setError("awfmGpuSearchHitsCompact: this batch does not take the seed-order path on this image");
    return AwFmUnsupportedVersionError;
  }
  DeviceGuard guard(g->device);
  hipStream_t s = (hipStream_t)stream;
  SparseOut sparse;
  sparse.count = (unsigned *)dNumHits;
  sparse.cap = capacity;
  sparse.kmers = (unsigned *)dHitKmers;
  sparse.ranges = (ulonglong2 *)dHitRanges;
  const int did = g->amino ? aminoLookupSearch(g, s, dChars, fixedLength, numQueries, nullptr, nullptr, false, &sparse)
                           : orderedSearch(g, s, dChars, (const unsigned long long *)dOffsets, fixedLength, numQueries, nullptr, nullptr,
// ... 174 lines not shown
  hipLaunchKernelGGL(mergeBucketRunsKernel, dim3(nb * kMergeParts + 4u), dim3(256), 0, (hipStream_t)stream, (const unsigned long long *)dReceived,
                     (const unsigned long long *)dSliceAt, dSliceStarts, numSlices, firstBucket, endBucket, buckets, (unsigned long long *)dRecords, dBucketStart);
  const hipError_t e = hipGetLastError();
  if (e != hipSuccess) {
    setError("awfmGpuMergeBucketRuns", e);
    return AwFmGeneralFailure;
  }
  return AwFmSuccess;
}

extern "C" enum AwFmReturnCode awfmGpuSearchOrderedRecords(AwFmGpuIndex *g, const uint64_t *dRecords, const uint32_t *dBucketStart, uint32_t firstBucket,
                                                           uint32_t endBucket, uint32_t fixedLength, uint64_t totalQueries, uint32_t *dOrderKmers,
                                                           struct AwFmSearchRange *dOrderRanges, void *stream) {
  return awfmGpuSearchOrderedRecordsCounts(g, dRecords, dBucketStart, firstBucket, endBucket, fixedLength, totalQueries, dOrderKmers, dOrderRanges, nullptr,
                                           stream);
}

extern "C" enum AwFmReturnCode awfmGpuSearchOrderedRecordsCounts(AwFmGpuIndex *g, const uint64_t *dRecords, const uint32_t *dBucketStart,
                                                                 uint32_t firstBucket, uint32_t endBucket, uint32_t fixedLength, uint64_t totalQueries,
                                                                 uint32_t *dOrderKmers, struct AwFmSearchRange *dOrderRanges, uint32_t *dOrderCounts,
                                                                 void *stream) {
  if (!g || !dRecords || !dBucketStart || !dOrderKmers || !dOrderRanges) {
    setError("awfmGpuSearchOrderedRecords: null argument");
    return AwFmNullPtrError;
  }
  unsigned depth = 0;
  const ulonglong2 *table = nullptr;
  BucketFormat fmt;
  if (!shardedFormat(g, fixedLength, totalQueries, &depth, &table, &fmt) || firstBucket >= endBucket || endBucket > (1u << fmt.bucketBits)) {
    setError("awfmGpuSearchOrderedRecords: buckets [first, end) of the records awfmGpuOrderKmers makes for this image and batch");
    return AwFmIllegalPositionError;
  }
  DeviceGuard guard(g->device);
  hipStream_t s = (hipStream_t)stream;
  std::lock_guard<std::mutex> lock(g->orderMutex);
  fmt.firstBucket = firstBucket;
  fmt.endBucket = endBucket;
  if (orderBeginSlot(g, s) != hipSuccess) {
    setError("seed-order search: could not order the use of its scratch across streams");
    return AwFmGeneralFailure;
  }
  OrderSlotScope slotScope(g, s);
  if (!ensureOrderScratch(g, kOrderCounterBytes)) return AwFmAllocationFailure;
  unsigned *generalCount = (unsigned *)g->dOrder;
  AWFM_HIP_TRY(hipMemsetAsync(generalCount, 0, kOrderCounterBytes, s), AwFmGeneralFailure);
  for (int i = 0; i < 4; i++) g->orderTiming[i] = nullptr;
  SparseOut out;
  out.count = nullptr;
  out.cap = 0;
  out.kmers = (unsigned *)dOrderKmers;
  out.ranges = (ulonglong2 *)dOrderRanges;
  const bool pair = pairSteps(g);
  enum AwFmReturnCode rc;
#define SHARD_GO(NR, PR) \
  launchOrderedKernel<NR, false, PR, false, true>(g, s, fixedLength, depth, table, totalQueries, dRecords, generalCount, nullptr, dOrderCounts, nullptr, (const unsigned *)dBucketStart, fmt, &out)
  if (awfmImageNarrow(g)) rc = pair ? SHARD_GO(true, true) : SHARD_GO(true, false);
  else rc = pair ? SHARD_GO(false, true) : SHARD_GO(false, false);
#undef SHARD_GO
  if (rc != AwFmSuccess) return rc;
  AWFM_HIP_TRY(slotScope.end(), AwFmGeneralFailure);
  return AwFmSuccess;
}

extern "C" enum AwFmReturnCode awfmGpuSearchGeneralRecords(AwFmGpuIndex *g, const uint8_t *dChars, uint32_t fixedLength, uint64_t numQueries,
                                                           uint64_t firstNumber, uint64_t totalQueries, const uint64_t *dRecords,
                                                           const uint32_t *dBucketStart, uint32_t *dOrderKmers, struct AwFmSearchRange *dOrderRanges,
                                                           void *stream) {
  if (!g || !dChars || !dRecords || !dBucketStart || !dOrderKmers || !dOrderRanges) {
    setError("awfmGpuSearchGeneralRecords: null argument");
    return AwFmNullPtrError;
  }
  unsigned depth = 0;
  const ulonglong2 *table = nullptr;
  BucketFormat fmt;
  if (numQueries == 0 || firstNumber + numQueries > totalQueries || !shardedFormat(g, fixedLength, totalQueries, &depth, &table, &fmt)) {
    setError("awfmGpuSearchGeneralRecords: the shard awfmGpuOrderKmers was given");
    return AwFmIllegalPositionError;
  }
  DeviceGuard guard(g->device);
  hipStream_t s = (hipStream_t)stream;
  const unsigned bins = (1u << fmt.bucketBits) + 1u;
  const unsigned *leftCount = (const unsigned *)dBucketStart + bins + 1u;
  SparseOut out;
  out.count = nullptr;
  out.cap = 0;
  out.kmers = (unsigned *)dOrderKmers;
  out.ranges = (ulonglong2 *)dOrderRanges;
  const uint8_t *base = dChars - (size_t)firstNumber * fixedLength;
  const bool narrow = awfmImageNarrow(g);
  const unsigned grid = narrow ? residentGrid(g, searchKernel<false, 4, false, false, true, true>) : residentGrid(g, searchKernel<false, 4, false, false, false, true>);
  if (narrow)
    hipLaunchKernelGGL((searchKernel<false, 4, false, false, true, true>), dim3(grid), dim3(kThreads), 0, s, g->image->dev, base, (const unsigned long long *)nullptr, fixedLength,
                       (unsigned long long)(firstNumber + numQueries), (ulonglong2 *)nullptr, (unsigned *)nullptr, (unsigned long long *)nullptr,
                       (const unsigned char *)dRecords, 8u, 0u, (unsigned long long)numQueries, leftCount, out, (const unsigned *)nullptr, 0u);
  else
    hipLaunchKernelGGL((searchKernel<false, 4, false, false, false, true>), dim3(grid), dim3(kThreads), 0, s, g->image->dev, base, (const unsigned long long *)nullptr, fixedLength,
                       (unsigned long long)(firstNumber + numQueries), (ulonglong2 *)nullptr, (unsigned *)nullptr, (unsigned long long *)nullptr,
                       (const unsigned char *)dRecords, 8u, 0u, (unsigned long long)numQueries, leftCount, out, (const unsigned *)nullptr, 0u);
  AWFM_HIP_TRY(hipGetLastError(), AwFmGeneralFailure);
  return AwFmSuccess;
}
#undef SHARD_TRY

extern "C" enum AwFmReturnCode awfmGpuCompactHits(AwFmGpuIndex *g, const uint32_t *dCounts, const struct AwFmSearchRange *dRanges,
                                                  uint64_t numQueries, uint64_t *dFlagOffsets, void *dScratch, uint32_t *dHitKmers,
                                                  struct AwFmSearchRange *dHitRanges, uint32_t capacity, uint32_t *dNumHits,
                                                  void *stream) {
  if (!g || !dCounts || !dRanges || !dFlagOffsets || !dScratch || !dHitKmers || !dHitRanges || !dNumHits) {
// ... 180 lines not shown
```

### avxwindowfmindex_amd/csrc/awfm_ordered_kernel.h

```cpp
#ifndef AWFM_ORDERED_KERNEL_H
#define AWFM_ORDERED_KERNEL_H

#include "awfm_search_kernel.h"
#include "awfm_pair.h"

namespace {

__device__ __forceinline__ void decodeWord(unsigned word, unsigned &packed, unsigned &badBits) {
  unsigned t = (word >> 1) & 0x03030303u;
  t ^= (t >> 1) & 0x01010101u;
  const unsigned b0 = t & 0x01010101u, b1 = (t >> 1) & 0x01010101u, b01 = b0 & b1;
  const unsigned expect = 0x61616161u + (b0 << 1) + b1 * 6u + b01 * 11u;
  unsigned diff = ((word | 0x20202020u) ^ expect) & ~b01;
  diff |= diff >> 4;
  diff |= diff >> 2;
  diff |= diff >> 1;
  diff &= 0x01010101u;
  badBits = (diff & 1u) | ((diff >> 7) & 2u) | ((diff >> 14) & 4u) | ((diff >> 21) & 8u);
  packed = ((t & 3u) << 6) | ((t >> 4) & 0x30u) | ((t >> 14) & 0x0Cu) | (t >> 24);
}

__device__ __forceinline__ void decodeWordAny(unsigned word, unsigned countMask, unsigned &packed, unsigned &diffs) {
  unsigned t = (word >> 1) & 0x03030303u;
  t ^= (t >> 1) & 0x01010101u;
  const unsigned b01 = t & (t >> 1) & 0x01010101u;
  const unsigned expect = __builtin_amdgcn_perm(0u, 0x74676361u, t);
  diffs |= ((word | 0x20202020u) ^ expect) & ~b01 & countMask;
  packed = ((t & 3u) << 6) | ((t >> 4) & 0x30u) | ((t >> 14) & 0x0Cu) | (t >> 24);
}

__device__ __forceinline__ void decodeKmer(const unsigned char *__restrict__ chars, unsigned long long start, unsigned len,
                                           unsigned long long &codes, unsigned &bad) {
  const unsigned long long at = (unsigned long long)chars + start;
  typedef const unsigned __attribute__((address_space(1))) *GlobalWords;
  const GlobalWords first = (GlobalWords)(at & ~3ull);
  const unsigned shift = (unsigned)at & 3u;
  const unsigned numDwords = (shift + len + 3u) >> 2;
  unsigned dw[9];
#pragma unroll
  for (int j = 0; j < 9; j++) dw[j] = (unsigned)j < numDwords ? first[j] : 0u;
  codes = 0;
  bad = 0;
#pragma unroll
  for (int j = 0; j < 8; j++) {
    unsigned packed = 0, badBits = 0;
    if (4u * j < len) decodeWord(__builtin_amdgcn_alignbyte(dw[j + 1], dw[j], shift), packed, badBits);
    codes = (codes << 8) | packed;
    bad |= badBits << (4 * j);
  }
  codes >>= 2u * (32u - len);
  bad &= len >= 32u ? ~0u : ((1u << len) - 1u);
}

__device__ __forceinline__ unsigned startKey15(unsigned long long codes, unsigned len, unsigned depth) {
  const unsigned span = depth ? depth : len;
  const unsigned long long str = span >= 32u ? codes : (codes & ((1ull << (2u * span)) - 1ull));
  return 2u * span >= 15u ? (unsigned)(str >> (2u * span - 15u)) : (unsigned)(str << (15u - 2u * span));
// ... 863 lines not shown
        const unsigned up = __shfl_up(incl, off);
        if ((int)(threadIdx.x & 63u) >= off) incl += up;
      }
      if ((threadIdx.x & 63u) == 63u) sWave[threadIdx.x >> 6] = incl;
      __syncthreads();
      unsigned running = incl - sum;
      for (unsigned w = 0; w < (threadIdx.x >> 6); w++) running += sWave[w];
#pragma unroll
      for (unsigned j = 0; j < kPer; j++) {
        const unsigned e = threadIdx.x * kPer + j;
        if (e < bins) {
          sLoc[e] = running;
          sDst[e] = start[j] + got[j];
        }
        running += v[j];
      }
    }
    __syncthreads();
#pragma unroll
    for (unsigned j = 0; j < kWideItems; j++)
      if (where[j] != 0xFFFFFFFFu) sRec[sLoc[where[j] >> 16] + (where[j] & 0xFFFFu)] = rec[j];
    __syncthreads();
    for (unsigned b = (threadIdx.x >> 3); b < bins; b += kPartitionThreads / 8u) {
      const unsigned count = sCnt[b], loc = sLoc[b];
      if (count != 0u && count <= kLongRun) {
        ulonglong2 *dst = (ulonglong2 *)(out + sDst[b]);
        for (unsigned j = threadIdx.x & 7u; j < count; j += 8u) dst[j] = sRec[loc + j];
      } else if (count > kLongRun && (threadIdx.x & 7u) == 0u) {
        sLong[atomicAdd(&sNumLong, 1u)] = b;
      }
    }
    __syncthreads();
    const unsigned numLong = sNumLong;
    for (unsigned k = 0; k < numLong; k++) {
      const unsigned b = sLong[k], count = sCnt[b], loc = sLoc[b];
      ulonglong2 *dst = (ulonglong2 *)(out + sDst[b]);
      for (unsigned j = threadIdx.x; j < count; j += kPartitionThreads) dst[j] = sRec[loc + j];
    }
    __syncthreads();
    if (threadIdx.x == 0) sNumLong = 0u;
  }
}

constexpr int orderedThreads(bool pair) { return pair ? 256 : kThreads; }

constexpr unsigned kTouchLevels = 32;
struct OrderTouch {
  unsigned long long *seedLines;
  unsigned long long *deepLines;
  unsigned long long *pairLines;
  unsigned long long *nucLines;
  unsigned long long pairWords, nucWords;
  unsigned long long *hits;
};

template <bool VARLEN>
struct OrderSkip {
  __device__ __forceinline__ bool chosen() const { return false; }
};
template <>
struct OrderSkip<true> {
  const unsigned *sampleAlive = nullptr;
  unsigned samples = 0;
  __device__ __forceinline__ bool chosen() const { return lookupChosen(sampleAlive, samples, false); }
};

constexpr unsigned kTicketGroups = 4;
template <int G, bool NARROW, bool VARLEN, bool PAIR = false, bool TOUCH = false, bool BUCKET = false,
          bool LIST = false >
__global__ void __launch_bounds__(orderedThreads(PAIR)) __attribute__((amdgpu_num_sgpr(80), amdgpu_waves_per_eu(G >= 2 ? ((PAIR && !NARROW) || TOUCH || (G == 2 && !NARROW) ? 6 : (VARLEN || PAIR || BUCKET ? 7 : 8)) : 2, 8)))
    orderedSearchKernel(const DevIndex ix, const void *__restrict__ recs, const unsigned long long numRecs,
                        const unsigned *__restrict__ generalCount, const unsigned len, const unsigned depth,
                        const ulonglong2 *__restrict__ table, ulonglong2 *__restrict__ ranges,
                        unsigned *__restrict__ counts, unsigned *__restrict__ tickets,
                        const OrderTouch touch = OrderTouch(), const unsigned *__restrict__ bucketStart = nullptr,
                        const BucketFormat bucketFmt = BucketFormat(), const SparseOut sparse = SparseOut(),
                        const unsigned chunksPerTicket = 1u, const OrderSkip<VARLEN> skip = OrderSkip<VARLEN>()) {
  static_assert(!BUCKET || !VARLEN, "bucketed records are the 8-byte records of fixed-length batches");
  if (skip.chosen()) return;
  constexpr bool AHEAD = BUCKET;
  constexpr int S = (int)kSlices / G;
  typedef typename PositionType<NARROW>::type pos_t;
  __shared__ unsigned long long sC[24];
  __shared__ unsigned sMask[(kBlockMask + 1) * kSlices];
  __shared__ unsigned long long sSuper[!NARROW ? kMaxNucSuper * 4 : 1];
  __shared__ unsigned long long sPairC[PAIR ? 16 : 1];
  extern __shared__ unsigned sPairSuper[];
  static_assert(!PAIR || G == 4, "pair steps are written for 4 lanes per query");
  static_assert(!LIST || BUCKET, "the collected list belongs to the bucketed variant (the one that runs after encodeLookupKernel)");
  constexpr unsigned kHitBuffer = LIST ? 32 : 1;
  __shared__ unsigned sHitKmers[LIST ? orderedThreads(PAIR) / 64 : 1][kHitBuffer];
  __shared__ unsigned long long sHitRanges[LIST ? orderedThreads(PAIR) / 64 : 1][kHitBuffer][2];
  unsigned hitFill = 0;
  const unsigned long long coveredFirst = BUCKET && bucketFmt.endBucket != 0u ? (unsigned long long)bucketStart[bucketFmt.firstBucket] : 0ull;
  const unsigned long long coveredEnd = BUCKET ? (unsigned long long)bucketStart[bucketFmt.endBucket != 0u ? bucketFmt.endBucket : 1u << bucketFmt.bucketBits]
                                               : numRecs - (unsigned long long)*generalCount;
  if (BUCKET && coveredEnd == coveredFirst) return;
  __shared__ unsigned sHitLeft[LIST ? orderedThreads(PAIR) / 64 : 1], sWavesDone;
  if (LIST && threadIdx.x == 0) sWavesDone = 0u;
  if (threadIdx.x < 24) sC[threadIdx.x] = ix.prefixSums[threadIdx.x];
  stageMaskTable(sMask);
  nucStageSuper<NARROW>(ix, sSuper);
  if (PAIR) pairStageTables<NARROW, 16u>(ix, sPairC, sPairSuper);
  __syncthreads();

  struct Raw {
    unsigned long long a, b;
  };
  auto readRecord = [&](unsigned long long at, Raw &r) {
    if (BUCKET) {
      r.a = ((const unsigned long long *)recs)[at];
    } else {
      const ulonglong2 w = *(const ulonglong2 *)((const QueryRec *)recs + at);
      r.a = w.x;
      r.b = w.y;
    }
  };
  const unsigned gl = threadIdx.x % G;
  const unsigned firstSlice = gl * S;
  auto markLine = [&](unsigned long long *bits, unsigned long long line) {
    if (TOUCH && gl == 0) atomicOr(bits + (line >> 6), 1ull << (line & 63ull));
  };
  auto touchNuc = [&](unsigned level, unsigned long long sp, unsigned long long ep) {
    if (TOUCH) {
      unsigned long long *bits = touch.nucLines + (level < kTouchLevels ? level : kTouchLevels - 1u) * touch.nucWords;
      markLine(bits, ((sp - 1ull) >> kBlockShift) >> 1);
      markLine(bits, (ep >> kBlockShift) >> 1);
    }
  };
  auto touchPair = [&](unsigned level, unsigned long long sp, unsigned long long ep) {
    if (TOUCH) {
      unsigned long long *bits = touch.pairLines + (level < kTouchLevels ? level : kTouchLevels - 1u) * touch.pairWords;
      markLine(bits, (sp - 1ull) >> kBlockShift);
      markLine(bits, ep >> kBlockShift);
    }
  };
  const unsigned long long covered = coveredEnd - coveredFirst;
  const unsigned xcds = (gridDim.x & 7u) == 0u ? 8u : 1u;
  const unsigned xcd = xcds == 8u ? (blockIdx.x & 7u) : 0u;
  const unsigned blockInXcd = xcds == 8u ? (blockIdx.x >> 3) : blockIdx.x;
  const unsigned long long share = (covered + xcds - 1ull) / xcds;
  const unsigned long long begin = coveredFirst + share * xcd;
  const unsigned long long end = begin + share < coveredEnd ? begin + share : coveredEnd;
  constexpr unsigned kWaves = orderedThreads(PAIR) / 64, kChunk = 64 / G;
  const unsigned wave = threadIdx.x >> 6, lane = threadIdx.x & 63u;
  auto flushHits = [&]() {
    if (hitFill != 0u) {
      __builtin_amdgcn_fence(__ATOMIC_RELEASE, "wavefront");
      __builtin_amdgcn_wave_barrier();
      unsigned listBase = 0;
      if (lane == 0) listBase = atomicAdd(sparse.count, hitFill);
      listBase = (unsigned)__builtin_amdgcn_readfirstlane((int)listBase);
// ... 8 lines not shown
  };
  constexpr unsigned kCounters = kTicketGroups * kWaves;
  const unsigned counter = (blockInXcd % kTicketGroups) * kWaves + wave;
  unsigned *ticket = tickets + (xcd * kCounters + counter) * 64u;
  auto ticketBase = [&](unsigned t) -> unsigned long long {
    return begin + ((unsigned long long)t * kCounters + counter) * chunksPerTicket * kChunk;
  };
  unsigned drawn = 0;
  if (lane == 0) drawn = atomicAdd(ticket, 1u);
  unsigned long long ticketAt = ticketBase((unsigned)__builtin_amdgcn_readfirstlane((int)drawn));
  unsigned sub = 0;
  if (lane == 0) drawn = atomicAdd(ticket, 1u);
  auto nextChunk = [&]() -> unsigned long long {
    if (sub == chunksPerTicket) {
      ticketAt = ticketBase((unsigned)__builtin_amdgcn_readfirstlane((int)drawn));
      sub = 0;
      if (lane == 0) drawn = atomicAdd(ticket, 1u);
    }
    return ticketAt + (unsigned long long)(sub++) * kChunk;
  };
  unsigned long long base = nextChunk();
  unsigned long long baseNext = nextChunk();

  const unsigned long long tableMask = (1ull << (2u * depth)) - 1ull;
  Raw raw = {0ull, 0ull};
  if (base + lane / G < end) readRecord(base + lane / G, raw);
  const unsigned numBuckets = BUCKET ? (bucketFmt.endBucket != 0u ? bucketFmt.endBucket : 1u << bucketFmt.bucketBits) : 0u;
  unsigned waveBucket = 0, waveNext = 0;
  if (BUCKET && base < end) {
    unsigned lo = 0, hi = numBuckets - 1u;
    while (lo < hi) {
      const unsigned mid = (lo + hi + 1u) >> 1;
      if ((unsigned long long)bucketStart[mid] <= base) lo = mid;
      else hi = mid - 1u;
    }
    waveBucket = lo;
    waveNext = bucketStart[lo + 1u];
  }
  auto laneBucket = [&](unsigned long long chunkAt) -> unsigned {
    while ((unsigned long long)waveNext <= chunkAt && waveBucket + 1u < numBuckets) {
      waveBucket++;
      waveNext = bucketStart[waveBucket + 1u];
    }
    unsigned mine = waveBucket, nb = waveBucket, ns = waveNext;
    while ((unsigned long long)ns <= chunkAt + (kChunk - 1u) && nb + 1u < numBuckets) {
      nb++;
      mine = chunkAt + lane / G >= (unsigned long long)ns ? nb : mine;
      ns = bucketStart[nb + 1u];
    }
    return mine;
  };
  const bool rawEntries = table == ix.deepSeed && ix.deepNarrow != 0u;
  const bool dropByNext = PAIR && !VARLEN && rawEntries && ix.deepNext != 0u && len >= depth + 2u;
  auto tableEntry = [&](unsigned long long codes) -> ulonglong2 {
    const unsigned long long at = codes & tableMask;
    if (rawEntries) {
      unsigned next16;
      ulonglong2 r = deepSeedOpen(ix, at, ((const uint2 *)ix.deepSeed)[at], &next16);
      if (dropByNext && ((next16 >> ((unsigned)(codes >> (2u * depth)) & 15u)) & 1u) == 0u) r = make_ulonglong2(1ull, 0ull);
      return r;
    }
    return table == ix.deepSeed ? deepSeedEntry(ix, at) : table[at];
  };
  auto touchTable = [&](unsigned long long at) {
    if (TOUCH) markLine(table == ix.seed ? touch.seedLines : touch.deepLines, at >> (table == ix.deepSeed && ix.deepNarrow ? 4 : 3));
  };
  unsigned long long codesCur = 0, baseNext2 = 0;
  unsigned indexCur = 0;
  pos_t entrySpCur = 1, entryEpCur = 0;
  if (AHEAD) {
    baseNext2 = nextChunk();
    if (base < end) {
      const unsigned mine = laneBucket(base);
      codesCur = bucketCodes(bucketFmt, mine, raw.a >> bucketFmt.indexBits);
      indexCur = (unsigned)(raw.a & ((1ull << bucketFmt.indexBits) - 1ull));
      if (base + lane / G < end) {
        const ulonglong2 r = tableEntry(codesCur);
        entrySpCur = (pos_t)r.x;
        entryEpCur = (pos_t)r.y;
        touchTable(codesCur & tableMask);
      }
    }
    if (baseNext + lane / G < end) readRecord(baseNext + lane / G, raw);
  }
  while (base < end) {
    const unsigned long long q = base + lane / G;
    const bool live = q < end;
    pos_t sp = 1, ep = 0;
    int pos = -1;
    unsigned long long rem;
    unsigned long long codes;
    unsigned index;
    pos_t entrySp = 1, entryEp = 0;
    if (AHEAD) {
      codes = codesCur;
      index = indexCur;
      entrySp = entrySpCur;
      entryEp = entryEpCur;
      asm volatile("" : "+v"(entrySp), "+v"(entryEp));
      entrySpCur = 1;
      entryEpCur = 0;
      if (baseNext < end) {
        const unsigned mine = laneBucket(baseNext);
        asm volatile("" : "+v"(raw.a)::"memory");
        codesCur = bucketCodes(bucketFmt, mine, raw.a >> bucketFmt.indexBits);
        indexCur = (unsigned)(raw.a & ((1ull << bucketFmt.indexBits) - 1ull));
        if (baseNext + lane / G < end) {
          const ulonglong2 r = tableEntry(codesCur);
          entrySpCur = (pos_t)r.x;
          entryEpCur = (pos_t)r.y;
          touchTable(codesCur & tableMask);
        }
      }
      if (baseNext2 + lane / G < end) readRecord(baseNext2 + lane / G, raw);
    } else {
    asm volatile("" : "+v"(raw.a), "+v"(raw.b)::"memory");
    codes = BUCKET ? bucketCodes(bucketFmt, laneBucket(base), raw.a >> bucketFmt.indexBits) : raw.a;
    index = BUCKET ? (unsigned)(raw.a & ((1ull << bucketFmt.indexBits) - 1ull)) : (unsigned)raw.b;
    }
    const unsigned myLen = VARLEN ? (unsigned)(raw.b >> 32) : len;
    if (!AHEAD) {
    if (!VARLEN && live) {
      const ulonglong2 r = tableEntry(codes);
      entrySp = (pos_t)r.x;
      entryEp = (pos_t)r.y;
      touchTable(codes & tableMask);
    }
    if (baseNext + lane / G < end) readRecord(baseNext + lane / G, raw);
    }
    if (!VARLEN) {
      if (live) {
        sp = entrySp;
        ep = entryEp;
        pos = (int)(len - depth) - 1;
      }
      rem = codes >> (2u * depth);
    } else {
      const unsigned myDepth = orderStartDepth(myLen, ix.seedK, ix.deepK);
      if (live) {
        if (myDepth != 0u) {
          const unsigned long long at = codes & ((1ull << (2u * myDepth)) - 1ull);
          ulonglong2 r;
          if (myDepth == ix.seedK) {
            r = ix.seed[at];
          } else if (ix.deepNarrow != 0u) {
            unsigned next16;
            r = deepSeedOpen(ix, at, ((const uint2 *)ix.deepSeed)[at], &next16);
            if (PAIR && ix.deepNext != 0u && myLen >= myDepth + 2u && ((next16 >> ((unsigned)(codes >> (2u * myDepth)) & 15u)) & 1u) == 0u)
              r = make_ulonglong2(1ull, 0ull);
          } else {
            r = deepSeedEntry(ix, at);
          }
          if (TOUCH) markLine(myDepth == ix.seedK ? touch.seedLines : touch.deepLines, at >> (myDepth != ix.seedK && ix.deepNarrow ? 4 : 3));
          sp = (pos_t)r.x;
          ep = (pos_t)r.y;
          pos = (int)(myLen - myDepth) - 1;
        } else {
          const unsigned a = (unsigned)codes & 3u;
          sp = (pos_t)sC[a];
// ... 51 lines not shown
            sHitRanges[w][at][1] = (unsigned long long)ep;
          }
          hitFill = (unsigned)__builtin_amdgcn_readfirstlane((int)(hitFill + hits));
        }
      } else if (sparse.kmers) {
        if (mine && sparse.ranges) {
          sparse.kmers[at - coveredFirst] = index;
          sparse.ranges[at - coveredFirst] = sp <= ep ? make_ulonglong2((unsigned long long)sp, (unsigned long long)ep) : make_ulonglong2(1ull, 0ull);
          if (counts) counts[at - coveredFirst] = sp <= ep ? (unsigned)(ep - sp + (pos_t)1) : 0u;
        } else if (mine) {
          ((uint2 *)sparse.kmers)[at - coveredFirst] = make_uint2(index, sp <= ep ? (unsigned)(ep - sp + (pos_t)1) : 0u);
        }
      } else if (mine && sp <= ep) {
        if (ranges) ranges[index] = make_ulonglong2((unsigned long long)sp, (unsigned long long)ep);
        if (counts) counts[index] = (unsigned)(ep - sp + (pos_t)1);
      }
    }
    if (LIST && hitFill + 64u / G > kHitBuffer) flushHits();
    base = baseNext;
    if (AHEAD) {
      baseNext = baseNext2;
      baseNext2 = nextChunk();
    } else {
      baseNext = nextChunk();
    }
  }
  if (LIST) {
    const unsigned w = (unsigned)__builtin_amdgcn_readfirstlane((int)(threadIdx.x >> 6));
    if (lane == 0) sHitLeft[w] = hitFill;
    __builtin_amdgcn_fence(__ATOMIC_RELEASE, "workgroup");
    unsigned arrived = 0;
    if (lane == 0) arrived = atomicAdd(&sWavesDone, 1u);
    arrived = (unsigned)__builtin_amdgcn_readfirstlane((int)arrived);
    if (arrived == kWaves - 1u) {
      __builtin_amdgcn_fence(__ATOMIC_ACQUIRE, "workgroup");
      unsigned total = 0;
      for (unsigned v = 0; v < kWaves; v++) total += sHitLeft[v];
      if (total != 0u) {
        unsigned listBase = 0;
        if (lane == 0) listBase = atomicAdd(sparse.count, total);
        listBase = (unsigned)__builtin_amdgcn_readfirstlane((int)listBase);
        unsigned before = 0;
        for (unsigned v = 0; v < kWaves; v++) {
          const unsigned n = sHitLeft[v];
          if (lane < n && listBase + before + lane < sparse.cap) {
            sparse.kmers[listBase + before + lane] = sHitKmers[v][lane];
            sparse.ranges[listBase + before + lane] = make_ulonglong2(sHitRanges[v][lane][0], sHitRanges[v][lane][1]);
          }
          before += n;
        }
      }
    }
  }
}


template <bool NARROW>
__global__ void __launch_bounds__(orderedThreads(true)) __attribute__((amdgpu_num_sgpr(80)))
    deepNextKernel(const DevIndex ix, uint2 *__restrict__ table, const unsigned long long numEntries,
                   unsigned *__restrict__ bigBySp, unsigned *__restrict__ numBig) {
  constexpr int G = 4;
  constexpr int S = (int)kSlices / G;
  typedef typename PositionType<NARROW>::type pos_t;
  __shared__ unsigned long long sC[24];
  __shared__ unsigned sMask[(kBlockMask + 1) * kSlices];
  __shared__ unsigned long long sSuper[NARROW ? 1 : kMaxNucSuper * 4];
  __shared__ unsigned long long sPairC[16];
  extern __shared__ unsigned sPairSuper[];
  if (threadIdx.x < 24) sC[threadIdx.x] = ix.prefixSums[threadIdx.x];
  stageMaskTable(sMask);
  nucStageSuper<NARROW>(ix, sSuper);
  pairStageTables<NARROW, 16u>(ix, sPairC, sPairSuper);
  __syncthreads();
  const unsigned gl = threadIdx.x % G, lane = threadIdx.x & 63u;
  const unsigned firstSlice = gl * S;
  constexpr unsigned long long kChunk = 64 / G;
  const unsigned long long waveStride = (unsigned long long)gridDim.x * (blockDim.x / 64u) * kChunk;
  for (unsigned long long base = ((unsigned long long)blockIdx.x * (blockDim.x / 64u) + threadIdx.x / 64u) * kChunk; base < numEntries;
       base += waveStride) {
    const unsigned long long at = base + lane / G;
    const uint2 e = at < numEntries ? table[at] : make_uint2(1u, 0u);
    const bool some = NARROW ? e.y != 0u : (e.y & (kDeepWideLengthMask << 4)) != 0u;
    if (some) {
      ulonglong2 r;
      if (NARROW) r = make_ulonglong2((unsigned long long)e.x, (unsigned long long)e.x + e.y - 1ull);
      else r = deepSeedOpen(ix, at, e, nullptr);
      unsigned next16 = 0;
      for (unsigned code = 0; code < 16u; code++) {
        pos_t sp = (pos_t)r.x, ep = (pos_t)r.y;
        if (pairSearchStep<NARROW>(ix, sPairC, sPairSuper, sMask, gl, code, sp, ep) == kPairFlagged) {
          nucFastStep<G, NARROW>(ix, sC, sSuper, sMask, firstSlice, code & 3u, sp, ep);
          if (sp <= ep) nucFastStep<G, NARROW>(ix, sC, sSuper, sMask, firstSlice, code >> 2, sp, ep);
        }
        if (sp <= ep) next16 |= 1u << code;
      }
      if (gl == 0) {
        if (NARROW) {
          if (e.y >= 0xFFFFu) {
            bigBySp[e.x >> kDeepBigShift] = e.y;
            atomicAdd(numBig, 1u);
          }
          table[at] = make_uint2(e.x, (e.y < 0xFFFFu ? e.y : 0xFFFFu) | next16 << 16);
        } else {
          if (((e.y >> 4) & kDeepWideLengthMask) == kDeepWideLengthMask) atomicAdd(numBig, 1u);
          table[at] = make_uint2(e.x, (e.y & 0xFFFFu) | next16 << 16);
        }
// ... 53 lines not shown
```

### include/awfm_gpu.h

```cpp
#ifndef AWFM_GPU_H
#define AWFM_GPU_H

#include "AwFmIndex.h"

#ifdef __cplusplus
extern "C" {
#endif

typedef struct AwFmGpuIndex AwFmGpuIndex;

enum AwFmGpuKernel {
  AWFM_GPU_KERNEL_AUTO = 0,
  AWFM_GPU_KERNEL_GROUP8 = 1,
  AWFM_GPU_KERNEL_GROUP4 = 2,
  AWFM_GPU_KERNEL_GROUP2 = 3,
  AWFM_GPU_KERNEL_GROUP1 = 4
};

int awfmGpuDeviceCount(void);
const char *awfmGpuLastError(void);
enum AwFmReturnCode awfmGpuLastBatchStatus(void);


enum AwFmReturnCode awfmGpuIndexCreate(const struct AwFmIndex *index, int device, AwFmGpuIndex **out);
void awfmGpuIndexDestroy(AwFmGpuIndex *g);
AwFmGpuIndex *awfmGpuIndexAcquire(const struct AwFmIndex *index);
int awfmGpuIndexAcquireAll(const struct AwFmIndex *index, AwFmGpuIndex **out, int maxOut);
void awfmGpuIndexRelease(const struct AwFmIndex *index);
uint64_t awfmGpuIndexDeviceBytes(const AwFmGpuIndex *g);
int awfmGpuIndexDevice(const AwFmGpuIndex *g);
enum AwFmReturnCode awfmGpuIndexSetDeepSeed(AwFmGpuIndex *g, unsigned deepK);
unsigned awfmGpuIndexDeepSeedK(const AwFmGpuIndex *g);
double awfmGpuIndexDeepSeedBuildSeconds(const AwFmGpuIndex *g);
double awfmGpuIndexDeepSeedAllocSeconds(const AwFmGpuIndex *g);
uint64_t awfmGpuIndexDeepSeedTransientBytes(const AwFmGpuIndex *g);
enum AwFmReturnCode awfmGpuIndexSetDenseSa(AwFmGpuIndex *g, int enable);
int awfmGpuIndexHasDenseSa(const AwFmGpuIndex *g);
int awfmGpuIndexDescribe(const AwFmGpuIndex *g, char *out, int outBytes);
double awfmGpuIndexDenseSaBuildSeconds(const AwFmGpuIndex *g);
uint64_t awfmGpuIndexLengthTableBytes(const AwFmGpuIndex *g);
double awfmGpuIndexLengthTableBuildSeconds(const AwFmGpuIndex *g);
enum AwFmReturnCode awfmGpuIndexSetPairImage(AwFmGpuIndex *g, int enable);
int awfmGpuIndexHasPairImage(const AwFmGpuIndex *g);
enum AwFmReturnCode awfmLocalPositions(const struct AwFmIndex *index, const uint64_t *positions, uint64_t numPositions,
                                       uint32_t *sequenceNumbers, uint64_t *localPositions, uint64_t *numIllegalOut,
                                       unsigned threads);
enum AwFmReturnCode awfmGpuIndexSetRecordTable(AwFmGpuIndex *g, const uint64_t *sequenceEndPositions, uint64_t numRecords);
uint32_t awfmGpuIndexNumRecords(const AwFmGpuIndex *g);
void awfmGpuIndexSetKernel(AwFmGpuIndex *g, enum AwFmGpuKernel kernel);
void awfmGpuIndexSetWide(AwFmGpuIndex *g, int wide);
int awfmGpuIndexIsWide(const AwFmGpuIndex *g);

enum AwFmReturnCode awfmGpuCreateIndex(struct AwFmIndex **index, const struct AwFmIndexConfiguration *config,
                                       const uint8_t *sequence, uint64_t sequenceLength, int sequenceOnDevice,
                                       const char *fileSrc, int device);

enum AwFmReturnCode awfmGpuSearch(AwFmGpuIndex *g, const uint8_t *dChars, const uint64_t *dOffsets,
                                  uint32_t fixedLength, uint64_t numQueries, struct AwFmSearchRange *dRanges,
                                  uint32_t *dCounts, void *stream);

enum AwFmReturnCode awfmLongestSuffixMatches(const struct AwFmIndex *index, const uint8_t *chars, const uint64_t *starts,
                                             const uint64_t *ends, uint32_t fixedLength, uint64_t numQueries, uint32_t minLength,
                                             uint32_t *matchLengths, struct AwFmSearchRange *ranges, uint32_t *counts,
                                             unsigned threads);
enum AwFmReturnCode awfmGpuLongestSuffixMatches(AwFmGpuIndex *g, const uint8_t *dChars, const uint64_t *dStarts,
                                                const uint64_t *dEnds, uint32_t fixedLength, uint64_t numQueries,
                                                uint32_t minLength, uint32_t *dMatchLengths, struct AwFmSearchRange *dRanges,
                                                uint32_t *dCounts, void *stream);

#define AWFM_EDIT_NONE 0xFFFFFFFFu
enum AwFmReturnCode awfmOneSubstitutionSearch(const struct AwFmIndex *index, const uint8_t *chars, const uint64_t *offsets,
                                              uint32_t fixedLength, uint64_t numQueries, int includeExact, uint32_t *hitQueries,
                                              uint32_t *hitEdits, struct AwFmSearchRange *hitRanges, uint64_t capacity,
                                              uint64_t *numHits, uint32_t *variantsPerQuery, uint64_t *occurrencesPerQuery,
                                              unsigned threads);
enum AwFmReturnCode awfmGpuOneSubstitutionSearch(AwFmGpuIndex *g, const uint8_t *dChars, const uint64_t *dOffsets,
                                                 uint32_t fixedLength, uint64_t numQueries, int includeExact,
                                                 uint32_t *dHitQueries, uint32_t *dHitEdits, struct AwFmSearchRange *dHitRanges,
                                                 uint64_t capacity, uint64_t *dNumHits, uint32_t *dVariantsPerQuery,
                                                 uint64_t *dOccurrencesPerQuery, void *stream);

enum AwFmReturnCode awfmGpuSearchHits(AwFmGpuIndex *g, const uint8_t *dChars, const uint64_t *dOffsets,
                                      uint32_t fixedLength, uint64_t numQueries, struct AwFmSearchRange *dRanges,
                                      uint32_t *dCounts, void *stream);
enum AwFmReturnCode awfmGpuSearchHitsSparse(AwFmGpuIndex *g, const uint8_t *dChars, const uint64_t *dOffsets,
                                            uint32_t fixedLength, uint64_t numQueries, struct AwFmSearchRange *dRanges,
                                            uint32_t *dCounts, void *stream);
enum AwFmReturnCode awfmGpuSearchHitsCompact(AwFmGpuIndex *g, const uint8_t *dChars, const uint64_t *dOffsets,
                                             uint32_t fixedLength, uint64_t numQueries, int packed, uint32_t *dHitKmers,
                                             struct AwFmSearchRange *dHitRanges, uint32_t capacity, uint32_t *dNumHits,
                                             void *stream);
enum AwFmReturnCode awfmGpuSearchHitsInOrder(AwFmGpuIndex *g, const uint8_t *dChars, const uint64_t *dOffsets,
                                             uint32_t fixedLength, uint64_t numQueries, int packed, uint32_t *dOrderKmers,
                                             struct AwFmSearchRange *dOrderRanges, void *stream);
// ... 169 lines not shown
  uint64_t *numMapped;
};
enum AwFmReturnCode awfmScoreChainsAffine(const struct AwFmVerifyInputs *in, uint64_t numReads, uint32_t maxCandidates, uint32_t bandPad,
                                          uint32_t maxDrift, const struct AwFmAlignScoring *scoring, uint32_t minScore, uint32_t mapqCap,
                                          const uint8_t *text, uint64_t length, const uint64_t *sequenceEnds, uint64_t numRecords,
                                          enum AwFmAlphabetType alphabet, const struct AwFmSlotScoreOutputs *out, unsigned threads);
enum AwFmReturnCode awfmGpuScoreChainsAffine(AwFmGpuIndex *g, const struct AwFmVerifyInputs *dIn, uint64_t numReads, uint32_t maxCandidates,
                                             uint32_t bandPad, uint32_t maxDrift, const struct AwFmAlignScoring *scoring, uint32_t minScore,
                                             uint32_t mapqCap, const struct AwFmSlotScoreOutputs *dOut, void *stream);

#define AWFM_WINDOW_MAX_WIDTH 4096u
#define AWFM_WINDOW_MAX_LENGTH 4096u
struct AwFmWindowInputs {
  const uint8_t *readChars;
  uint64_t numReadChars;
  const uint64_t *readOffsets;
  const uint32_t *windowSequences;
  const uint64_t *windowBegins;
  const uint64_t *windowEnds;
};
struct AwFmWindowOutputs {
  uint32_t *scores;
  uint32_t *readBegins;
  uint32_t *readEnds;
  uint64_t *textBegins;
  uint64_t *textEnds;
  uint32_t *sequences, *chainAnchors, *chainReadBegins, *chainReadEnds;
  int64_t *chainBeginDiagonals, *chainEndDiagonals;
  uint64_t *numUnscored;
  uint64_t *numFound;
};
enum AwFmReturnCode awfmScoreWindowsAffine(const struct AwFmWindowInputs *in, uint64_t numReads, const struct AwFmAlignScoring *scoring,
                                           uint32_t minScore, uint32_t slotStride, uint32_t slotColumn, const uint8_t *text, uint64_t length,
                                           const uint64_t *sequenceEnds, uint64_t numRecords, enum AwFmAlphabetType alphabet,
                                           const struct AwFmWindowOutputs *out, unsigned threads);
uint64_t awfmGpuScoreWindowsAffineScratchBytes(const AwFmGpuIndex *g, uint32_t maxLength);
enum AwFmReturnCode awfmGpuScoreWindowsAffine(AwFmGpuIndex *g, const struct AwFmWindowInputs *dIn, uint64_t numReads,
                                              const struct AwFmAlignScoring *scoring, uint32_t minScore, uint32_t slotStride,
                                              uint32_t slotColumn, uint32_t maxLength, const struct AwFmWindowOutputs *dOut, void *dScratch,
                                              void *stream);

void awfmGpuIndexSetOrdered(AwFmGpuIndex *g, int mode);
int awfmGpuSearchHitsIsOrdered(const AwFmGpuIndex *g, int hasOffsets, uint32_t fixedLength, uint64_t numQueries);
void awfmGpuStreamRetire(AwFmGpuIndex *g, void *stream);

double awfmGpuLastOrderedKernelMs(AwFmGpuIndex *g);
int awfmGpuLastOrderedKernelIsLookup(AwFmGpuIndex *g);
int awfmGpuLastLookupFront(AwFmGpuIndex *g);
int awfmGpuLastSearchWasExactLookup(AwFmGpuIndex *g);
double awfmGpuLastOrderedSearchKernelMs(AwFmGpuIndex *g);
int awfmGpuOrderedKernelLog(AwFmGpuIndex *g, double *frontMs, double *kernelMs, int max);
uint64_t awfmGpuLastOrderedKept(AwFmGpuIndex *g);
void awfmGpuLastSecondWindow(AwFmGpuIndex *g, uint64_t out[2]);

enum AwFmReturnCode awfmGpuSearchTally(AwFmGpuIndex *g, const uint8_t *dChars, const uint64_t *dOffsets,
                                       uint32_t fixedLength, uint64_t numQueries, uint64_t tallyOut[4]);

enum AwFmReturnCode awfmGpuMixedLookupLineTally(AwFmGpuIndex *g, const uint8_t *dChars, const uint64_t *dOffsets,
                                                uint64_t numQueries, uint64_t tallyOut[8]);

enum AwFmReturnCode awfmGpuSearchHitsLineTally(AwFmGpuIndex *g, const uint8_t *dChars, const uint64_t *dOffsets,
                                               uint32_t fixedLength, uint64_t numQueries, uint64_t tallyOut[8]);

uint64_t awfmGpuScanScratchBytes(uint64_t numQueries);
enum AwFmReturnCode awfmGpuHitOffsets(AwFmGpuIndex *g, const struct AwFmSearchRange *dRanges, uint64_t numQueries,
                                      uint64_t *dHitOffsets, void *dScratch, uint64_t *totalHits, void *stream);
enum AwFmReturnCode awfmGpuHitOffsetsFromCounts(AwFmGpuIndex *g, const uint32_t *dCounts, uint64_t numQueries,
                                                uint64_t *dHitOffsets, void *dScratch, uint64_t *totalHits, void *stream);

enum AwFmReturnCode awfmGpuHitOffsetsOnDevice(AwFmGpuIndex *g, const uint32_t *dCounts, const struct AwFmSearchRange *dRanges,
                                              uint64_t numQueries, uint64_t *dHitOffsets, void *dScratch, void *stream);
enum AwFmReturnCode awfmGpuLocateOnDevice(AwFmGpuIndex *g, const struct AwFmSearchRange *dRanges, const uint64_t *dHitOffsets,
                                          uint64_t numQueries, uint64_t capacityHits, uint64_t *dPositions, void *stream);

enum AwFmReturnCode awfmGpuLocate(AwFmGpuIndex *g, const struct AwFmSearchRange *dRanges,
                                  const uint64_t *dHitOffsets, uint64_t numQueries, uint64_t totalHits,
                                  uint64_t *dPositions, void *stream);

enum AwFmReturnCode awfmGpuLocateTo(AwFmGpuIndex *g, const struct AwFmSearchRange *dRanges,
                                    const uint64_t *dHitOffsets, uint64_t numQueries, uint64_t totalHits,
                                    uint64_t *dPositions, uint64_t *outPositions, void *stream);

enum AwFmReturnCode awfmGpuLocateWindow(AwFmGpuIndex *g, const struct AwFmSearchRange *dRanges, const uint64_t *dHitOffsets,
                                        uint64_t queryBegin, uint64_t queryEnd, uint64_t hitBegin, uint64_t hitEnd,
                                        uint64_t *dPositions, uint64_t *outPositions, void *stream);

void awfmGpuAosLastStages(double out[10]);
double awfmHostCopyGBs(unsigned threads, uint64_t bytes);

void *awfmGpuPinnedBuffer(AwFmGpuIndex *g, int slot, uint64_t bytes);
void awfmGpuAosLock(AwFmGpuIndex *g);
void awfmGpuAosUnlock(AwFmGpuIndex *g);

enum AwFmReturnCode awfmGpuCountHost(AwFmGpuIndex *g, const uint8_t *chars, const uint64_t *offsets,
                                     uint32_t fixedLength, uint64_t numQueries, struct AwFmSearchRange *ranges,
                                     uint32_t *counts);
enum AwFmReturnCode awfmGpuLocateHost(AwFmGpuIndex *g, const uint8_t *chars, const uint64_t *offsets,
                                      uint32_t fixedLength, uint64_t numQueries, struct AwFmSearchRange *ranges,
                                      uint64_t *hitOffsets, uint64_t **positions);

enum AwFmReturnCode awfmGpuLocateHostLocal(AwFmGpuIndex *g, const uint8_t *chars, const uint64_t *offsets, uint32_t fixedLength,
                                           uint64_t numQueries, struct AwFmSearchRange *ranges, uint64_t *hitOffsets,
                                           uint32_t **sequenceNumbers, uint64_t **localPositions, uint64_t *numIllegal);

typedef int (*AwFmGpuHitWindowSink)(void *user, uint64_t queryBegin, uint64_t queryEnd, uint64_t hitBegin, uint64_t hitEnd,
                                    const uint64_t *positions);
// ... 84 lines not shown
```

Measured before the change: 38170.

## Add compact nibble-packed deep seed table for bucketed pair ordered search

Builds a compact version of the deep k-mer seed table that stores per-entry range lengths as 4-bit fields, with a per-sub-block start position and prefix sums to rebuild suffix array ranges. A dedicated kernel variant reads one 16-byte chunk per lookup instead of the wider raw entry, and falls back to the full table for irregular sub-blocks. The goal is to cut memory traffic and cache footprint for the seed lookups. It costs extra device memory, a table build step, fallback counters with atomics, and more code paths.

```diff
diff --git a/avxwindowfmindex_amd/_lib.py b/avxwindowfmindex_amd/_lib.py
--- a/avxwindowfmindex_amd/_lib.py
+++ b/avxwindowfmindex_amd/_lib.py
@@ -27,7 +27,7 @@
 GPU_SYMBOLS = [
     "awfmGpuDeviceCount", "awfmGpuLastError", "awfmGpuIndexCreate", "awfmGpuIndexDestroy", "awfmGpuIndexAcquire", "awfmGpuIndexAcquireAll",
     "awfmGpuIndexRelease", "awfmGpuIndexDeviceBytes", "awfmGpuIndexDevice", "awfmGpuIndexSetKernel", "awfmGpuIndexSetWide", "awfmGpuIndexIsWide", "awfmGpuLastBatchStatus", "awfmGpuIndexSetDeepSeed", "awfmGpuIndexSetDenseSa", "awfmGpuPinnedBuffer", "awfmGpuLocateHostWindows", "awfmGpuLocateWindow", "awfmGpuAosLock",
-    "awfmGpuAosUnlock", "awfmGpuSearch", "awfmGpuSearchHits", "awfmGpuSearchHitsSparse", "awfmGpuIndexSetOrdered", "awfmGpuSearchHitsIsOrdered", "awfmGpuLastOrderedKernelMs", "awfmGpuLastOrderedKernelIsLookup", "awfmGpuLastOrderedKept", "awfmGpuLastSecondWindow",
+    "awfmGpuAosUnlock", "awfmGpuSearch", "awfmGpuSearchHits", "awfmGpuSearchHitsSparse", "awfmGpuIndexSetOrdered", "awfmGpuSearchHitsIsOrdered", "awfmGpuLastOrderedKernelMs", "awfmGpuLastOrderedKernelIsLookup", "awfmGpuLastOrderedKept", "awfmGpuLastSecondWindow", "awfmGpuLastCompactTable", "awfmGpuIndexCompactTableBytes", "awfmGpuIndexCompactTableBuildSeconds",
     "awfmGpuScanScratchBytes", "awfmGpuHitOffsets", "awfmGpuHitOffsetsFromCounts", "awfmGpuLocate", "awfmGpuCountHost", "awfmGpuLocateHost",
     "awfmGpuCreateIndex", "awfmGpuSearchTally", "awfmGpuSynthText", "awfmGpuSynthRandomQueries", "awfmGpuSynthPlantedQueries",
     "awfmGpuSynthMixedLengths", "awfmGpuSynthMixedQueries", "awfmGpuSynthGenomeText", "awfmGpuSynthPlantedQueriesClean",
@@ -218,6 +218,9 @@
         "awfmGpuLastOrderedKernelIsLookup": (C.c_int, [vp]),
         "awfmGpuLastOrderedKept": (C.c_uint64, [vp]),
         "awfmGpuLastSecondWindow": (None, [vp, C.POINTER(C.c_uint64 * 2)]),
+        "awfmGpuLastCompactTable": (None, [vp, C.POINTER(C.c_uint64 * 2)]),
+        "awfmGpuIndexCompactTableBytes": (C.c_uint64, [vp]),
+        "awfmGpuIndexCompactTableBuildSeconds": (C.c_double, [vp]),
         "awfmGpuIndexSetDeepSeed": (C.c_int, [vp, C.c_uint]),
         "awfmGpuIndexSetDenseSa": (C.c_int, [vp, C.c_int]),
         "awfmGpuIndexSetPairImage": (C.c_int, [vp, C.c_int]),
diff --git a/avxwindowfmindex_amd/api.py b/avxwindowfmindex_amd/api.py
--- a/avxwindowfmindex_amd/api.py
+++ b/avxwindowfmindex_amd/api.py
@@ -821,6 +821,10 @@
     def length_tables(self):
         return (int(_lib.lib().awfmGpuIndexLengthTableBytes(self.handle)), float(_lib.lib().awfmGpuIndexLengthTableBuildSeconds(self.handle)))
 
+    @property
+    def compact_table(self):
+        return (int(_lib.lib().awfmGpuIndexCompactTableBytes(self.handle)), float(_lib.lib().awfmGpuIndexCompactTableBuildSeconds(self.handle)))
+
     def mixed_lookup_line_tally(self, d_chars, d_offsets, n):
         out = (C.c_uint64 * 8)()
         _check("awfmGpuMixedLookupLineTally", _lib.lib().awfmGpuMixedLookupLineTally(self.handle, d_chars, d_offsets, n, C.byref(out)))
@@ -1195,6 +1199,11 @@
         _lib.lib().awfmGpuLastSecondWindow(self.handle, C.byref(out))
         return int(out[0]), int(out[1])
 
+    def last_compact_table(self):
+        out = (C.c_uint64 * 2)()
+        _lib.lib().awfmGpuLastCompactTable(self.handle, C.byref(out))
+        return int(out[0]), int(out[1])
+
     def last_ordered_kernel_is_lookup(self):
         return bool(_lib.lib().awfmGpuLastOrderedKernelIsLookup(self.handle))
 
diff --git a/avxwindowfmindex_amd/csrc/awfm_compact_table.h b/avxwindowfmindex_amd/csrc/awfm_compact_table.h
--- /dev/null
+++ b/avxwindowfmindex_amd/csrc/awfm_compact_table.h
@@ -0,0 +1,91 @@
+#ifndef AWFM_COMPACT_TABLE_H
+#define AWFM_COMPACT_TABLE_H
+
+#include <stdint.h>
+
+#if defined(__HIPCC__) || defined(__CUDACC__)
+#define AWFM_COMPACT_HD __host__ __device__ inline
+#else
+#define AWFM_COMPACT_HD inline
+#endif
+
+enum {
+  kCompactSubCodes = 32,
+  kCompactSubsPerLine = 6,
+  kCompactLineCodes = 192,
+  kCompactLineWords = 32,
+  kCompactStartWord = 24,
+  kCompactFlagsWord = 30,
+  kCompactEscape = 15
+};
+#define kCompactIrregular 0xFFFFFFFFu
+
+enum { kCompactEmpty = 0, kCompactAnswered = 1, kCompactFallBack = 2 };
+
+AWFM_COMPACT_HD uint64_t awfmCompactLines(uint64_t numEntries) { return (numEntries + kCompactLineCodes - 1u) / kCompactLineCodes; }
+AWFM_COMPACT_HD uint64_t awfmCompactBytes(uint64_t numEntries) { return awfmCompactLines(numEntries) * (kCompactLineWords * 4u); }
+
+AWFM_COMPACT_HD void awfmCompactWhere(uint32_t i, uint32_t *line, uint32_t *sub, uint32_t *field) {
+  const uint32_t block = i >> 5;
+  *line = block / kCompactSubsPerLine;
+  *sub = block - *line * kCompactSubsPerLine;
+  *field = i & 31u;
+}
+AWFM_COMPACT_HD uint32_t awfmCompactSubWord(uint32_t sub) { return sub * 4u; }
+
+AWFM_COMPACT_HD uint32_t awfmCompactField(uint32_t w0, uint32_t w1, uint32_t w2, uint32_t w3, uint32_t field) {
+  const uint32_t d = field >> 3;
+  const uint32_t w = d == 0u ? w0 : d == 1u ? w1 : d == 2u ? w2 : w3;
+  return (w >> (4u * (field & 7u))) & 15u;
+}
+AWFM_COMPACT_HD uint32_t awfmCompactPrefix(uint32_t w0, uint32_t w1, uint32_t w2, uint32_t w3, uint32_t field) {
+  const uint32_t d = field >> 3;
+  const uint32_t part = (1u << (4u * (field & 7u))) - 1u;
+  const uint32_t m0 = d == 0u ? part : 0xFFFFFFFFu;
+  const uint32_t m1 = d == 1u ? part : (d > 1u ? 0xFFFFFFFFu : 0u);
+  const uint32_t m2 = d == 2u ? part : (d > 2u ? 0xFFFFFFFFu : 0u);
+  const uint32_t m3 = d == 3u ? part : 0u;
+  const uint32_t a = w0 & m0, b = w1 & m1, c = w2 & m2, e = w3 & m3;
+  const uint32_t low = 0x0F0F0F0Fu;
+  uint32_t s = (a & low) + ((a >> 4) & low) + (b & low) + ((b >> 4) & low) + (c & low) + ((c >> 4) & low) + (e & low) + ((e >> 4) & low);
+  s = (s & 0x00FF00FFu) + ((s >> 8) & 0x00FF00FFu);
+  return (s + (s >> 16)) & 0xFFFFu;
+}
+
+AWFM_COMPACT_HD int awfmCompactOpen(uint32_t w0, uint32_t w1, uint32_t w2, uint32_t w3, uint32_t start, uint32_t field, uint32_t *sp,
+                                    uint32_t *length) {
+  const uint32_t mine = awfmCompactField(w0, w1, w2, w3, field);
+  if (mine == 0u) return kCompactEmpty;
+  if (start == kCompactIrregular) return kCompactFallBack;
+  *sp = start + awfmCompactPrefix(w0, w1, w2, w3, field);
+  *length = mine;
+  return kCompactAnswered;
+}
+
+struct AwfmCompactPacker {
+  uint32_t w[4];
+  uint32_t start;
+  uint32_t sum;
+  uint32_t any, regular;
+};
+AWFM_COMPACT_HD void awfmCompactPackBegin(AwfmCompactPacker *p) {
+  p->w[0] = p->w[1] = p->w[2] = p->w[3] = 0u;
+  p->start = 0u;
+  p->sum = 0u;
+  p->any = 0u;
+  p->regular = 1u;
+}
+AWFM_COMPACT_HD void awfmCompactPackAdd(AwfmCompactPacker *p, uint32_t field, uint32_t sp, uint64_t length) {
+  if (length == 0u) return;
+  if (!p->any) {
+    p->any = 1u;
+    p->start = sp - p->sum;
+  }
+  if (length >= (uint64_t)kCompactEscape || sp != p->start + p->sum) p->regular = 0u;
+  const uint32_t nibble = length >= (uint64_t)kCompactEscape ? (uint32_t)kCompactEscape : (uint32_t)length;
+  p->w[field >> 3] |= nibble << (4u * (field & 7u));
+  p->sum += nibble;
+}
+AWFM_COMPACT_HD uint32_t awfmCompactPackStart(const AwfmCompactPacker *p) { return p->regular ? p->start : kCompactIrregular; }
+
+#endif
diff --git a/avxwindowfmindex_amd/csrc/awfm_device.h b/avxwindowfmindex_amd/csrc/awfm_device.h
--- a/avxwindowfmindex_amd/csrc/awfm_device.h
+++ b/avxwindowfmindex_amd/csrc/awfm_device.h
@@ -775,6 +775,13 @@
   void *dLengthBig = nullptr;
   uint64_t lengthTableBytes = 0;
   double lengthTableBuildSeconds = 0.0;
+  std::mutex compactMutex;
+  void *dCompactTable = nullptr;
+  bool compactTried = false;
+  unsigned compactRetryIn = 0;
+  uint64_t compactTableBytes = 0;
+  uint64_t compactIrregular = 0;
+  double compactTableBuildSeconds = 0.0;
   void *dDenseSa = nullptr;
   bool denseWide = false;
   uint64_t denseSaBytes = 0;
@@ -872,6 +879,7 @@
   bool orderLookupFused = false;
   const unsigned *orderFusedKeptAt = nullptr;
   const unsigned *orderKeptAt = nullptr;
+  const unsigned *orderCompactAt = nullptr;
   struct LookupPredict {
     unsigned long long *verdictHost = nullptr;
     unsigned searches = 0;
diff --git a/avxwindowfmindex_amd/csrc/awfm_gpu_image.hip b/avxwindowfmindex_amd/csrc/awfm_gpu_image.hip
--- a/avxwindowfmindex_amd/csrc/awfm_gpu_image.hip
+++ b/avxwindowfmindex_amd/csrc/awfm_gpu_image.hip
@@ -411,7 +411,7 @@
       if (image->pendingAccel.dense) (void)hipFree(image->pendingAccel.dense);
       awfmGpuStreamStateFree(image);
       void *owned[] = {image->dBlocks, image->dSuper, image->dSeed, image->dSa, image->dPrefix, image->dDeepSeed, image->dDeepBig,
-                       image->dDenseSa, image->dLengthTable, image->dLengthBig, image->dPairBlocks, image->dPairSuper,
+                       image->dDenseSa, image->dLengthTable, image->dLengthBig, image->dCompactTable, image->dPairBlocks, image->dPairSuper,
                        image->dPairSuper32, image->dPairC, image->dRecords, image->dText};
       for (void *p : owned)
         if (p) (void)hipFree(p);
@@ -556,7 +556,7 @@
 }
 
 static uint64_t imageBytes(const AwFmGpuImage *image) {
-  return image->deviceBytes + image->deepSeedBytes + image->denseSaBytes + image->pairBytes + image->lengthTableBytes + image->recordBytes + image->textBytes;
+  return image->deviceBytes + image->deepSeedBytes + image->denseSaBytes + image->pairBytes + image->lengthTableBytes + image->compactTableBytes + image->recordBytes + image->textBytes;
 }
 uint64_t awfmGpuIndexDeviceBytes(const AwFmGpuIndex *g) { return g && !g->lane ? imageBytes(g->image) : 0; }
 
@@ -610,6 +610,15 @@
   return AwFmSuccess;
 }
 static void installDeepSeed(AwFmGpuImage *image, AwFmGpuImage::PendingAccel *from) {
+  {
+    std::lock_guard<std::mutex> lock(image->compactMutex);
+    if (image->dCompactTable) (void)hipFree(image->dCompactTable);
+    image->dCompactTable = nullptr;
+    image->compactTableBytes = 0;
+    image->compactIrregular = 0;
+    image->compactTried = false;
+    image->compactRetryIn = 0;
+  }
   image->dDeepSeed = from->deepTable;
   image->dDeepBig = from->deepBig;
   image->deepSeedBytes = from->deepBytes + from->deepBigBytes;
@@ -755,6 +764,8 @@
   text += image->dev.deepK ? "deeper table depth " + std::to_string(image->dev.deepK) + (image->dev.deepNext ? " with next-step bits; " : "; ") : "deeper table no; ";
   text += image->dDenseSa ? "full suffix array yes; " : "full suffix array no; ";
   if (!g->amino) text += image->dLengthTable ? "tables per k-mer length 1.." + std::to_string(image->lengthDepths) + "; " : "tables per k-mer length not built (the first large mixed-length batch builds them); ";
+  if (image->dCompactTable)
+    text += "compact deeper table " + std::to_string(image->compactTableBytes) + " bytes, " + std::to_string(image->compactIrregular) + " sub-blocks fall back; ";
   text += awfmGpuDescribeRecordTable(image);
   text += awfmGpuDescribeText(image);
   if (!image->accelNotes.empty()) text += "notes: " + image->accelNotes;
@@ -766,5 +777,7 @@
 }
 uint64_t awfmGpuIndexLengthTableBytes(const AwFmGpuIndex *g) { return g ? g->image->lengthTableBytes : 0; }
 double awfmGpuIndexLengthTableBuildSeconds(const AwFmGpuIndex *g) { return g ? g->image->lengthTableBuildSeconds : 0.0; }
-
-}
+uint64_t awfmGpuIndexCompactTableBytes(const AwFmGpuIndex *g) { return g ? g->image->compactTableBytes : 0; }
+double awfmGpuIndexCompactTableBuildSeconds(const AwFmGpuIndex *g) { return g ? g->image->compactTableBuildSeconds : 0.0; }
+
+}
diff --git a/avxwindowfmindex_amd/csrc/awfm_gpu_ordered.hip b/avxwindowfmindex_amd/csrc/awfm_gpu_ordered.hip
--- a/avxwindowfmindex_amd/csrc/awfm_gpu_ordered.hip
+++ b/avxwindowfmindex_amd/csrc/awfm_gpu_ordered.hip
@@ -47,14 +47,20 @@
                                         unsigned long long nq, const void *recs, const unsigned *generalCount, ulonglong2 *rng,
                                         uint32_t *dCounts, const OrderTouch *touch = nullptr, const unsigned *bucketStart = nullptr,
                                         const BucketFormat bucketFmt = BucketFormat(), const SparseOut *sparse = nullptr,
-                                        const unsigned *skipSampleAlive = nullptr, unsigned skipSamples = 0u) {
+                                        const unsigned *skipSampleAlive = nullptr, unsigned skipSamples = 0u,
+                                        const unsigned *compact = nullptr, unsigned *compactCounters = nullptr) {
   constexpr int G = 4;
+  constexpr bool kHasCompactTwin = NARROW && !VARLEN && PAIR && BUCKET && !LIST;
+  const bool useCompact = kHasCompactTwin && compact != nullptr && compactCounters != nullptr;
   const bool superInLds = PAIR && NARROW && awfmPairSuperInLds(g);
   const size_t lds = superInLds ? (size_t)g->image->dev.numPairSuper * 64u : 0u;
   DevIndex dev = g->image->dev;
   dev.pairSuperInLds = superInLds ? 1u : 0u;
   constexpr int threads = orderedThreads(PAIR);
-  unsigned grid = residentGrid(g, orderedSearchKernel<G, NARROW, VARLEN, PAIR, TOUCH, BUCKET, LIST>, lds, threads);
+  unsigned grid = 0;
+  if constexpr (kHasCompactTwin)
+    if (useCompact) grid = residentGrid(g, compactOrderedKernel<TOUCH>, lds, threads);
+  if (!useCompact) grid = residentGrid(g, orderedSearchKernel<G, NARROW, VARLEN, PAIR, TOUCH, BUCKET, LIST>, lds, threads);
   const unsigned long long blocks = (nq + threads / G - 1) / (threads / G);
   if (blocks < grid) grid = (unsigned)blocks;
   if (grid >= 8u) grid &= ~7u;
@@ -64,6 +70,13 @@
     skip.sampleAlive = skipSampleAlive;
     skip.samples = skipSamples;
   }
+  g->orderCompactAt = useCompact ? compactCounters : nullptr;
+  if constexpr (kHasCompactTwin)
+    if (useCompact)
+      AWFM_LAUNCH_WITH_EVENTS((compactOrderedKernel<TOUCH>), dim3(grid ? grid : 1u), dim3(threads), (unsigned)lds, s, timed ? g->orderTiming[2] : nullptr,
+                              timed ? g->orderTiming[3] : nullptr, dev, recs, nq, generalCount, len, depth, table, rng, dCounts, (unsigned *)generalCount + 64,
+                              touch ? *touch : OrderTouch(), bucketStart, bucketFmt, sparse ? *sparse : SparseOut(), 2u, compact, compactCounters);
+  if (!useCompact)
   AWFM_LAUNCH_WITH_EVENTS((orderedSearchKernel<G, NARROW, VARLEN, PAIR, TOUCH, BUCKET, LIST>), dim3(grid ? grid : 1u), dim3(threads), (unsigned)lds, s,
                         timed ? g->orderTiming[2] : nullptr, timed ? g->orderTiming[3] : nullptr, dev, recs, nq, generalCount, len, depth, table,
                         rng, dCounts, (unsigned *)generalCount + 64, touch ? *touch : OrderTouch(), bucketStart, bucketFmt,
@@ -111,17 +124,18 @@
 enum AwFmReturnCode launchBucketed(AwFmGpuIndex *g, hipStream_t s, const uint8_t *dChars, uint32_t len, unsigned depth,
                                    const ulonglong2 *table, unsigned long long nq, const void *recs, const unsigned *bucketStart,
                                    const BucketFormat &fmt, const unsigned *generalCount, ulonglong2 *rng, uint32_t *dCounts,
-                                   bool packed, const OrderTouch *touch, const SparseOut *sparse, bool countRecords = false) {
+                                   bool packed, const OrderTouch *touch, const SparseOut *sparse, bool countRecords = false,
+                                   const unsigned *compact = nullptr, unsigned *compactCounters = nullptr) {
   const bool pair = pairSteps(g);
   enum AwFmReturnCode rc;
   if (touch)
-    rc = pair ? launchOrderedKernel<NARROW, false, true, true, true>(g, s, len, depth, table, nq, recs, generalCount, rng, dCounts, touch, bucketStart, fmt)
+    rc = pair ? launchOrderedKernel<NARROW, false, true, true, true>(g, s, len, depth, table, nq, recs, generalCount, rng, dCounts, touch, bucketStart, fmt, nullptr, nullptr, 0u, compact, compactCounters)
               : launchOrderedKernel<NARROW, false, false, true, true>(g, s, len, depth, table, nq, recs, generalCount, rng, dCounts, touch, bucketStart, fmt);
   else if (sparse && sparse->count)
     rc = pair ? launchOrderedKernel<NARROW, false, true, false, true, true>(g, s, len, depth, table, nq, recs, generalCount, rng, dCounts, nullptr, bucketStart, fmt, sparse)
               : launchOrderedKernel<NARROW, false, false, false, true, true>(g, s, len, depth, table, nq, recs, generalCount, rng, dCounts, nullptr, bucketStart, fmt, sparse);
   else
-    rc = pair ? launchOrderedKernel<NARROW, false, true, false, true>(g, s, len, depth, table, nq, recs, generalCount, rng, dCounts, nullptr, bucketStart, fmt, sparse)
+    rc = pair ? launchOrderedKernel<NARROW, false, true, false, true>(g, s, len, depth, table, nq, recs, generalCount, rng, dCounts, nullptr, bucketStart, fmt, sparse, nullptr, 0u, compact, compactCounters)
               : launchOrderedKernel<NARROW, false, false, false, true>(g, s, len, depth, table, nq, recs, generalCount, rng, dCounts, nullptr, bucketStart, fmt, sparse);
   if (rc != AwFmSuccess || packed || countRecords) return rc;
   return launchLeftover<NARROW, false>(g, s, dChars, nullptr, len, nq, rng, dCounts, recs, 8u, 0u, generalCount, sparse);
@@ -572,6 +586,119 @@
   if (p.searches == 0u) p.searches = 1u;
   p.lastFront = front;
   return p.searches | ((unsigned)front << 22) | ((fixedLength & 63u) << 24);
+}
+
+namespace {
+__global__ void __launch_bounds__(256) compactBuildKernel(const uint2 *__restrict__ table, const unsigned long long numEntries, const unsigned hasNext,
+                                                          unsigned *__restrict__ out, const unsigned long long numSubs,
+                                                          unsigned long long *__restrict__ irregular) {
+  const unsigned long long stride = (unsigned long long)gridDim.x * 256ull;
+  for (unsigned long long first = (unsigned long long)blockIdx.x * 256ull; first < numSubs; first += stride) {
+    const unsigned long long b = first + threadIdx.x;
+    bool bad = false;
+    if (b < numSubs) {
+      const unsigned long long at = b * kCompactSubCodes;
+      AwfmCompactPacker packer;
+      awfmCompactPackBegin(&packer);
+      for (unsigned f = 0; f < (unsigned)kCompactSubCodes; f += 2u) {
+        uint4 two = make_uint4(0u, 0u, 0u, 0u);
+        if (at + f + 1u < numEntries) two = *(const uint4 *)(table + at + f);
+        awfmCompactPackAdd(&packer, f, two.x, hasNext ? (two.y & 0xFFFFu) : two.y);
+        awfmCompactPackAdd(&packer, f + 1u, two.z, hasNext ? (two.w & 0xFFFFu) : two.w);
+      }
+      const unsigned long long line = b / kCompactSubsPerLine;
+      const unsigned sub = (unsigned)(b - line * kCompactSubsPerLine);
+      unsigned *words = out + line * kCompactLineWords;
+      *(uint4 *)(words + awfmCompactSubWord(sub)) = make_uint4(packer.w[0], packer.w[1], packer.w[2], packer.w[3]);
+      words[kCompactStartWord + sub] = awfmCompactPackStart(&packer);
+      if (packer.regular) atomicOr(words + kCompactFlagsWord, 1u << sub);
+      bad = !packer.regular;
+    }
+    const unsigned n = (unsigned)__popcll(__ballot(bad));
+    if ((threadIdx.x & 63u) == 0u && n) atomicAdd(irregular, (unsigned long long)n);
+  }
+}
+}
+
+static bool compactTableApplies(const AwFmGpuIndex *g, const ulonglong2 *table, unsigned depth) {
+  const DevIndex &dev = g->image->dev;
+  return !g->amino && awfmImageNarrow(g) && table != nullptr && table == dev.deepSeed && dev.deepNarrow == 1u && depth == dev.deepK && depth >= 1u &&
+         depth <= 16u && dev.bwtLength < 0xFFFFFFFFull && pairSteps(g);
+}
+
+static const unsigned *ensureCompactTable(AwFmGpuIndex *g) {
+  AwFmGpuImage *im = g->image;
+  std::lock_guard<std::mutex> lock(im->compactMutex);
+  if (im->dCompactTable) return (const unsigned *)im->dCompactTable;
+  if (im->compactTried && (++im->compactRetryIn & 63u) != 0u) return nullptr;
+  im->compactTried = true;
+  const unsigned long long numEntries = 1ull << (2u * im->dev.deepK);
+  const uint64_t bytes = awfmCompactBytes(numEntries);
+  {
+    size_t freeBytes = 0, totalBytes = 0;
+    if (hipMemGetInfo(&freeBytes, &totalBytes) != hipSuccess || (uint64_t)freeBytes / 3u < bytes) {
+      (void)hipGetLastError();
+      return nullptr;
+    }
+  }
+  struct timespec t0, t1;
+  clock_gettime(CLOCK_MONOTONIC, &t0);
+  void *table = nullptr;
+  unsigned long long *dIrregular = nullptr;
+  if (hipMalloc(&table, bytes) != hipSuccess || hipMalloc((void **)&dIrregular, 16) != hipSuccess) {
+    (void)hipGetLastError();
+    if (table) (void)hipFree(table);
+    return nullptr;
+  }
+  unsigned long long irregular = 0;
+  const unsigned long long numSubs = awfmCompactLines(numEntries) * kCompactSubsPerLine;
+  bool ok = awfmGpuSetupMemset(table, 0, bytes) == hipSuccess && awfmGpuSetupMemset(dIrregular, 0, 16) == hipSuccess;
+  if (ok) {
+    const unsigned long long tiles = (numSubs + 255ull) / 256ull;
+    const unsigned grid = (unsigned)(tiles < (unsigned long long)g->numCUs * 32u ? tiles : (unsigned long long)g->numCUs * 32u);
+    hipLaunchKernelGGL(compactBuildKernel, dim3(grid ? grid : 1u), dim3(256), 0, awfmGpuSetupStream, (const uint2 *)im->dev.deepSeed, numEntries,
+                       im->dev.deepNext, (unsigned *)table, numSubs, dIrregular);
+    ok = hipGetLastError() == hipSuccess && awfmGpuSetupSync() == hipSuccess && awfmGpuSetupToHost(&irregular, dIrregular, 8) == hipSuccess;
+  }
+  (void)hipFree(dIrregular);
+  if (!ok) {
+    (void)hipGetLastError();
+    (void)hipFree(table);
+    return nullptr;
+  }
+  clock_gettime(CLOCK_MONOTONIC, &t1);
+  im->dCompactTable = table;
+  im->compactTableBytes = bytes;
+  im->compactIrregular = irregular;
+  im->compactTableBuildSeconds = (double)(t1.tv_sec - t0.tv_sec) + 1e-9 * (double)(t1.tv_nsec - t0.tv_nsec);
+  if (awfmKnob(AWFM_KNOB_VERBOSE))
+    fprintf(stderr, "[awfm compact table] depth %u: %.3f GB in %.3f s; %llu of %llu sub-blocks fall back\n", im->dev.deepK, (double)bytes * 1e-9,
+            im->compactTableBuildSeconds, irregular, numSubs);
+  return (const unsigned *)table;
+}
+
+static const unsigned *compactTableFor(AwFmGpuIndex *g, const ulonglong2 *table, unsigned depth, bool wanted) {
+  if (!compactTableApplies(g, table, depth)) return nullptr;
+  if (const char *env = awfmGpuDiag("compact_table")) wanted = atoi(env) != 0;
+  return wanted ? ensureCompactTable(g) : nullptr;
+}
+
+extern "C" void awfmGpuLastCompactTable(AwFmGpuIndex *g, uint64_t out[2]) {
+  if (!out) return;
+  out[0] = out[1] = 0;
+  if (!g) return;
+  std::lock_guard<std::mutex> lock(g->orderMutex);
+  if (!g->orderCompactAt) return;
+  DeviceGuard guard(g->device);
+  unsigned words[kFusedCounters * 16u];
+  if (hipDeviceSynchronize() != hipSuccess || hipMemcpy(words, g->orderCompactAt, sizeof words, hipMemcpyDeviceToHost) != hipSuccess) {
+    (void)hipGetLastError();
+    return;
+  }
+  for (unsigned i = 0; i < kFusedCounters; i++) {
+    out[0] += words[i * 16u + 4u];
+    out[1] += words[i * 16u + 5u];
+  }
 }
 
 static int bucketedSearch(AwFmGpuIndex *g, hipStream_t s, const uint8_t *dChars, uint32_t fixedLength, unsigned depth,
@@ -758,9 +885,13 @@
   BUCKET_TRY(hipGetLastError());
   const SparseOut countOut{nullptr, 0u, (unsigned *)(w + countInAt), nullptr};
   const SparseOut *results = countRecords ? &countOut : sparse;
+  const unsigned *compact = nullptr;
+  g->orderCompactAt = nullptr;
+  if (!(results && results->count) && !lookupFirst && (!touch || touch->compactLines)) compact = compactTableFor(g, table, depth, false);
+  unsigned *compactCounters = (unsigned *)(w + kKeptAt);
   const enum AwFmReturnCode rc =
-      narrow ? launchBucketed<true>(g, s, dChars, fixedLength, depth, table, nq, recs, bucketStart, fmt, generalCount, rng, dCounts, packed, touch, results, countRecords)
-                         : launchBucketed<false>(g, s, dChars, fixedLength, depth, table, nq, recs, bucketStart, fmt, generalCount, rng, dCounts, packed, touch, results, countRecords);
+      narrow ? launchBucketed<true>(g, s, dChars, fixedLength, depth, table, nq, recs, bucketStart, fmt, generalCount, rng, dCounts, packed, touch, results, countRecords, compact, compactCounters)
+                         : launchBucketed<false>(g, s, dChars, fixedLength, depth, table, nq, recs, bucketStart, fmt, generalCount, rng, dCounts, packed, touch, results, countRecords, compact, compactCounters);
   if (rc != AwFmSuccess) return -(int)rc;
   if (countRecords) {
     const unsigned *ordered = bucketStart + (1u << fmt.bucketBits);
@@ -1303,7 +1434,16 @@
   const uint64_t seedWords = (g->image->dev.seedLen * 16u / 128u + 64u) / 64u;
   const uint64_t deepWords = g->image->dev.deepK ? ((1ull << (2u * g->image->dev.deepK)) * (g->image->dev.deepNarrow ? 8u : 16u) / 128u + 64u) / 64u : 1u;
   const uint64_t pairWords = (g->image->numBlocks + 64u) / 64u, nucWords = (g->image->numBlocks / 2u + 64u) / 64u;
-  const uint64_t words = seedWords + deepWords + (uint64_t)kTouchLevels * (pairWords + nucWords) + 8u;
+  unsigned compactDepth = 0;
+  const ulonglong2 *compactFrom = nullptr;
+  bool compactTally = !dOffsets && orderedApplies(g, false, fixedLength, numQueries, &compactDepth, &compactFrom) &&
+                      bucketFits(fixedLength, bucketFormat(compactDepth, numQueries)) && compactTableApplies(g, compactFrom, compactDepth);
+  if (compactTally) {
+    const char *env = awfmGpuDiag("compact_table");
+    compactTally = env && atoi(env) != 0;
+  }
+  const uint64_t compactWords = compactTally ? (awfmCompactLines(1ull << (2u * compactDepth)) + 64u) / 64u : 0u;
+  const uint64_t words = seedWords + deepWords + (uint64_t)kTouchLevels * (pairWords + nucWords) + compactWords + 16u;
   unsigned long long *bits = nullptr;
   if (hipMalloc((void **)&bits, words * 8u) != hipSuccess) {
     (void)hipGetLastError();
@@ -1319,10 +1459,30 @@
   touch.nucLines = touch.pairLines + (uint64_t)kTouchLevels * pairWords;
   touch.pairWords = pairWords;
   touch.nucWords = nucWords;
-  unsigned long long *sums = touch.nucLines + (uint64_t)kTouchLevels * nucWords;
+  unsigned long long *compactLines = touch.nucLines + (uint64_t)kTouchLevels * nucWords;
+  unsigned long long *sums = compactLines + compactWords;
   touch.hits = sums;
   uint64_t recordBytes = 0;
   hipError_t e = hipMemsetAsync(bits, 0, words * 8u, s);
+  if (e == hipSuccess && compactTally) {
+    constexpr unsigned kSamples = 16384;
+    const char *lookupEnv = awfmKnob(AWFM_KNOB_LOOKUP_FIRST);
+    const bool lookupWanted = lookupEnv ? atoi(lookupEnv) != 0 : numQueries >= (1ull << 20);
+    if (lookupWanted && lookupEnv && atoi(lookupEnv) == 1) {
+      compactTally = false;
+    } else if (lookupWanted && numQueries >= kSamples) {
+      const unsigned useNext = g->image->dev.deepNext != 0u && pairSteps(g) && fixedLength >= compactDepth + 2u ? 1u : 0u;
+      hipLaunchKernelGGL(lookupPrepKernel<false>, dim3(kSamples / 256u), dim3(256), 0, s, g->image->dev, dChars, fixedLength, compactDepth, useNext,
+                         (unsigned long long)numQueries, kSamples, sums + 8, sums + 10, (uint4 *)nullptr, 0u, (uint4 *)nullptr, 0u, SparseOut(),
+                         (unsigned long long *)nullptr, 0u);
+      unsigned long long alive = 0;
+      e = hipGetLastError();
+      if (e == hipSuccess) e = hipMemcpyAsync(&alive, sums + 8, sizeof alive, hipMemcpyDeviceToHost, s);
+      if (e == hipSuccess) e = hipStreamSynchronize(s);
+      if (e == hipSuccess && (unsigned)alive * 4u < kSamples) compactTally = false;
+    }
+    if (compactTally) touch.compactLines = compactLines;
+  }
   if (e == hipSuccess) {
     const int did = orderedSearch(g, s, dChars, (const unsigned long long *)dOffsets, fixedLength, numQueries, nullptr, nullptr, false,
                                   false, &touch, &recordBytes, nullptr);
@@ -1336,6 +1496,7 @@
         {touch.nucLines, (uint64_t)kTouchLevels * nucWords}};
     for (int i = 0; i < 4; i++)
       hipLaunchKernelGGL(popcountWordsKernel, dim3(1024), dim3(256), 0, s, parts[i].from, (unsigned long long)parts[i].n, sums + 1 + i);
+    if (touch.compactLines) hipLaunchKernelGGL(popcountWordsKernel, dim3(1024), dim3(256), 0, s, compactLines, (unsigned long long)compactWords, sums + 5);
     e = hipGetLastError();
     if (e == hipSuccess) e = hipMemcpyAsync(host, sums, sizeof(host), hipMemcpyDeviceToHost, s);
     if (e == hipSuccess) e = hipMemcpyAsync(&generalCount, g->dOrder, sizeof(generalCount), hipMemcpyDeviceToHost, s);
@@ -1348,7 +1509,7 @@
   }
   if (rc != AwFmSuccess) return rc;
   tallyOut[0] = host[1];
-  tallyOut[1] = host[2];
+  tallyOut[1] = host[2] + host[5];
   tallyOut[2] = host[3];
   tallyOut[3] = host[4];
   tallyOut[4] = numQueries - generalCount;
@@ -1629,8 +1790,11 @@
   out.ranges = (ulonglong2 *)dOrderRanges;
   const bool pair = pairSteps(g);
   enum AwFmReturnCode rc;
+  const unsigned *compact = compactTableFor(g, table, depth, false);
+  unsigned *compactCounters = generalCount + 102400u / 4u;
+  static_assert(102400u + kFusedCounters * 64u <= kOrderCounterBytes, "counter block");
 #define SHARD_GO(NR, PR) \
-  launchOrderedKernel<NR, false, PR, false, true>(g, s, fixedLength, depth, table, totalQueries, dRecords, generalCount, nullptr, dOrderCounts, nullptr, (const unsigned *)dBucketStart, fmt, &out)
+  launchOrderedKernel<NR, false, PR, false, true>(g, s, fixedLength, depth, table, totalQueries, dRecords, generalCount, nullptr, dOrderCounts, nullptr, (const unsigned *)dBucketStart, fmt, &out, nullptr, 0u, compact, compactCounters)
   if (awfmImageNarrow(g)) rc = pair ? SHARD_GO(true, true) : SHARD_GO(true, false);
   else rc = pair ? SHARD_GO(false, true) : SHARD_GO(false, false);
 #undef SHARD_GO
diff --git a/avxwindowfmindex_amd/csrc/awfm_ordered_kernel.h b/avxwindowfmindex_amd/csrc/awfm_ordered_kernel.h
--- a/avxwindowfmindex_amd/csrc/awfm_ordered_kernel.h
+++ b/avxwindowfmindex_amd/csrc/awfm_ordered_kernel.h
@@ -3,6 +3,7 @@
 
 #include "awfm_search_kernel.h"
 #include "awfm_pair.h"
+#include "awfm_compact_table.h"
 
 namespace {
 
@@ -972,6 +973,7 @@
   unsigned long long *nucLines;
   unsigned long long pairWords, nucWords;
   unsigned long long *hits;
+  unsigned long long *compactLines = nullptr;
 };
 
 template <bool VARLEN>
@@ -986,16 +988,19 @@
 };
 
 constexpr unsigned kTicketGroups = 4;
-template <int G, bool NARROW, bool VARLEN, bool PAIR = false, bool TOUCH = false, bool BUCKET = false,
-          bool LIST = false >
-__global__ void __launch_bounds__(orderedThreads(PAIR)) __attribute__((amdgpu_num_sgpr(80), amdgpu_waves_per_eu(G >= 2 ? ((PAIR && !NARROW) || TOUCH || (G == 2 && !NARROW) ? 6 : (VARLEN || PAIR || BUCKET ? 7 : 8)) : 2, 8)))
-    orderedSearchKernel(const DevIndex ix, const void *__restrict__ recs, const unsigned long long numRecs,
-                        const unsigned *__restrict__ generalCount, const unsigned len, const unsigned depth,
-                        const ulonglong2 *__restrict__ table, ulonglong2 *__restrict__ ranges,
-                        unsigned *__restrict__ counts, unsigned *__restrict__ tickets,
-                        const OrderTouch touch = OrderTouch(), const unsigned *__restrict__ bucketStart = nullptr,
-                        const BucketFormat bucketFmt = BucketFormat(), const SparseOut sparse = SparseOut(),
-                        const unsigned chunksPerTicket = 1u, const OrderSkip<VARLEN> skip = OrderSkip<VARLEN>()) {
+#define AWFM_ORDERED_ATTRIBUTES \
+  __launch_bounds__(orderedThreads(PAIR)) __attribute__((amdgpu_num_sgpr(80), amdgpu_waves_per_eu(G >= 2 ? ((PAIR && !NARROW) || TOUCH || (G == 2 && !NARROW) ? 6 : (VARLEN || PAIR || BUCKET ? 7 : 8)) : 2, 8)))
+template <int G, bool NARROW, bool VARLEN, bool PAIR, bool TOUCH, bool BUCKET, bool LIST, bool COMPACT>
+__device__ __forceinline__ void
+    orderedSearchBody(const DevIndex &ix, const void *__restrict__ recs, const unsigned long long numRecs,
+                      const unsigned *__restrict__ generalCount, const unsigned len, const unsigned depth,
+                      const ulonglong2 *__restrict__ table, ulonglong2 *__restrict__ ranges,
+                      unsigned *__restrict__ counts, unsigned *__restrict__ tickets,
+                      const OrderTouch touch, const unsigned *__restrict__ bucketStart,
+                      const BucketFormat bucketFmt, const SparseOut sparse,
+                      const unsigned chunksPerTicket, const OrderSkip<VARLEN> skip,
+                      const unsigned *__restrict__ compact, unsigned *__restrict__ compactCounters) {
+  static_assert(!COMPACT || (G == 4 && !VARLEN && PAIR && BUCKET && !LIST && NARROW), "the compact table: bucketed pair variant of images below 2^32 positions");
   static_assert(!BUCKET || !VARLEN, "bucketed records are the 8-byte records of fixed-length batches");
   if (skip.chosen()) return;
   constexpr bool AHEAD = BUCKET;
@@ -1018,6 +1023,8 @@
   if (BUCKET && coveredEnd == coveredFirst) return;
   __shared__ unsigned sHitLeft[LIST ? orderedThreads(PAIR) / 64 : 1], sWavesDone;
   if (LIST && threadIdx.x == 0) sWavesDone = 0u;
+  __shared__ unsigned sCompactFell[COMPACT ? orderedThreads(PAIR) / 64 : 1];
+  if (COMPACT && threadIdx.x < orderedThreads(PAIR) / 64) sCompactFell[threadIdx.x] = 0u;
   if (threadIdx.x < 24) sC[threadIdx.x] = ix.prefixSums[threadIdx.x];
   stageMaskTable(sMask);
   nucStageSuper<NARROW>(ix, sSuper);
@@ -1132,8 +1139,22 @@
   };
   const bool rawEntries = table == ix.deepSeed && ix.deepNarrow != 0u;
   const bool dropByNext = PAIR && !VARLEN && rawEntries && ix.deepNext != 0u && len >= depth + 2u;
+  unsigned compactLookups = 0;
   auto tableEntry = [&](unsigned long long codes) -> ulonglong2 {
     const unsigned long long at = codes & tableMask;
+    if (COMPACT) {
+      unsigned line, sub, field, sp32 = 0, length32 = 0;
+      awfmCompactWhere((unsigned)at, &line, &sub, &field);
+      const unsigned *words = compact + (unsigned long long)line * kCompactLineWords;
+      const uint4 w = *(const uint4 *)(words + awfmCompactSubWord(sub));
+      const unsigned start = words[kCompactStartWord + sub];
+      const int how = awfmCompactOpen(w.x, w.y, w.z, w.w, start, field, &sp32, &length32);
+      if (TOUCH) markLine(touch.compactLines, line);
+      if (how == kCompactEmpty) return make_ulonglong2(1ull, 0ull);
+      if (how == kCompactAnswered) return make_ulonglong2((unsigned long long)sp32, (unsigned long long)sp32 + length32 - 1ull);
+      if (threadIdx.x % G == 0) atomicAdd(&sCompactFell[threadIdx.x >> 6], 1u);
+      if (TOUCH) markLine(touch.deepLines, at >> 4);
+    }
     if (rawEntries) {
       unsigned next16;
       ulonglong2 r = deepSeedOpen(ix, at, ((const uint2 *)ix.deepSeed)[at], &next16);
@@ -1143,7 +1164,7 @@
     return table == ix.deepSeed ? deepSeedEntry(ix, at) : table[at];
   };
   auto touchTable = [&](unsigned long long at) {
-    if (TOUCH) markLine(table == ix.seed ? touch.seedLines : touch.deepLines, at >> (table == ix.deepSeed && ix.deepNarrow ? 4 : 3));
+    if (TOUCH && !COMPACT) markLine(table == ix.seed ? touch.seedLines : touch.deepLines, at >> (table == ix.deepSeed && ix.deepNarrow ? 4 : 3));
   };
   unsigned long long codesCur = 0, baseNext2 = 0;
   unsigned indexCur = 0;
@@ -1154,6 +1175,7 @@
       const unsigned mine = laneBucket(base);
       codesCur = bucketCodes(bucketFmt, mine, raw.a >> bucketFmt.indexBits);
       indexCur = (unsigned)(raw.a & ((1ull << bucketFmt.indexBits) - 1ull));
+      if (COMPACT) compactLookups += end - base < (unsigned long long)kChunk ? (unsigned)(end - base) : kChunk;
       if (base + lane / G < end) {
         const ulonglong2 r = tableEntry(codesCur);
         entrySpCur = (pos_t)r.x;
@@ -1185,6 +1207,7 @@
         asm volatile("" : "+v"(raw.a)::"memory");
         codesCur = bucketCodes(bucketFmt, mine, raw.a >> bucketFmt.indexBits);
         indexCur = (unsigned)(raw.a & ((1ull << bucketFmt.indexBits) - 1ull));
+        if (COMPACT) compactLookups += end - baseNext < (unsigned long long)kChunk ? (unsigned)(end - baseNext) : kChunk;
         if (baseNext + lane / G < end) {
           const ulonglong2 r = tableEntry(codesCur);
           entrySpCur = (pos_t)r.x;
@@ -1342,6 +1365,43 @@
       }
     }
   }
+  if (COMPACT) {
+    __builtin_amdgcn_fence(__ATOMIC_RELEASE, "wavefront");
+    __builtin_amdgcn_wave_barrier();
+    if (lane == 0 && compactLookups != 0u) {
+      const unsigned fell = sCompactFell[wave];
+      unsigned *line = compactCounters + ((blockIdx.x * kWaves + wave) % kFusedCounters) * 16u;
+      atomicAdd(line + 4, compactLookups - fell);
+      if (fell) atomicAdd(line + 5, fell);
+    }
+  }
+}
+
+template <int G, bool NARROW, bool VARLEN, bool PAIR = false, bool TOUCH = false, bool BUCKET = false,
+          bool LIST = false >
+__global__ void AWFM_ORDERED_ATTRIBUTES
+    orderedSearchKernel(const DevIndex ix, const void *__restrict__ recs, const unsigned long long numRecs,
+                        const unsigned *__restrict__ generalCount, const unsigned len, const unsigned depth,
+                        const ulonglong2 *__restrict__ table, ulonglong2 *__restrict__ ranges,
+                        unsigned *__restrict__ counts, unsigned *__restrict__ tickets,
+                        const OrderTouch touch = OrderTouch(), const unsigned *__restrict__ bucketStart = nullptr,
+                        const BucketFormat bucketFmt = BucketFormat(), const SparseOut sparse = SparseOut(),
+                        const unsigned chunksPerTicket = 1u, const OrderSkip<VARLEN> skip = OrderSkip<VARLEN>()) {
+  orderedSearchBody<G, NARROW, VARLEN, PAIR, TOUCH, BUCKET, LIST, false>(ix, recs, numRecs, generalCount, len, depth, table, ranges, counts, tickets, touch,
+                                                                         bucketStart, bucketFmt, sparse, chunksPerTicket, skip, nullptr, nullptr);
+}
+
+template <bool TOUCH = false>
+__global__ void __launch_bounds__(orderedThreads(true)) __attribute__((amdgpu_num_sgpr(80), amdgpu_waves_per_eu(TOUCH ? 6 : 7, 8)))
+    compactOrderedKernel(const DevIndex ix, const void *__restrict__ recs, const unsigned long long numRecs,
+                         const unsigned *__restrict__ generalCount, const unsigned len, const unsigned depth,
+                         const ulonglong2 *__restrict__ table, ulonglong2 *__restrict__ ranges,
+                         unsigned *__restrict__ counts, unsigned *__restrict__ tickets, const OrderTouch touch,
+                         const unsigned *__restrict__ bucketStart, const BucketFormat bucketFmt, const SparseOut sparse,
+                         const unsigned chunksPerTicket, const unsigned *__restrict__ compact, unsigned *__restrict__ compactCounters) {
+  orderedSearchBody<4, true, false, true, TOUCH, true, false, true>(ix, recs, numRecs, generalCount, len, depth, table, ranges, counts, tickets, touch,
+                                                                      bucketStart, bucketFmt, sparse, chunksPerTicket, OrderSkip<false>(), compact,
+                                                                      compactCounters);
 }
 
 
diff --git a/include/awfm_gpu.h b/include/awfm_gpu.h
--- a/include/awfm_gpu.h
+++ b/include/awfm_gpu.h
@@ -40,6 +40,8 @@
 double awfmGpuIndexDenseSaBuildSeconds(const AwFmGpuIndex *g);
 uint64_t awfmGpuIndexLengthTableBytes(const AwFmGpuIndex *g);
 double awfmGpuIndexLengthTableBuildSeconds(const AwFmGpuIndex *g);
+uint64_t awfmGpuIndexCompactTableBytes(const AwFmGpuIndex *g);
+double awfmGpuIndexCompactTableBuildSeconds(const AwFmGpuIndex *g);
 enum AwFmReturnCode awfmGpuIndexSetPairImage(AwFmGpuIndex *g, int enable);
 int awfmGpuIndexHasPairImage(const AwFmGpuIndex *g);
 enum AwFmReturnCode awfmLocalPositions(const struct AwFmIndex *index, const uint64_t *positions, uint64_t numPositions,
@@ -315,6 +317,7 @@
 int awfmGpuOrderedKernelLog(AwFmGpuIndex *g, double *frontMs, double *kernelMs, int max);
 uint64_t awfmGpuLastOrderedKept(AwFmGpuIndex *g);
 void awfmGpuLastSecondWindow(AwFmGpuIndex *g, uint64_t out[2]);
+void awfmGpuLastCompactTable(AwFmGpuIndex *g, uint64_t out[2]);
 
 enum AwFmReturnCode awfmGpuSearchTally(AwFmGpuIndex *g, const uint8_t *dChars, const uint64_t *dOffsets,
                                        uint32_t fixedLength, uint64_t numQueries, uint64_t tallyOut[4]);
```

New measurement: 37080. -2.9%, worse.
